# caishiqing/voice-tts

Measured on AMD Instinct MI355X. Metric: audio_seconds_per_second, higher is better.
Workload: dtype bf16

## Files before the change

### include/ixtts_hip.h

```cpp
#ifndef IXTTS_HIP_H
#define IXTTS_HIP_H

#include <stddef.h>
#include <stdint.h>

#ifdef __cplusplus
extern "C" {
#endif

#define IXTTS_OK 0
#define IXTTS_ERR_ARG (-1)
#define IXTTS_ERR_HIP (-2)
#define IXTTS_ERR_STATE (-3)
#define IXTTS_ERR_NOMEM (-4)
#define IXTTS_ERR_NAME (-5)

const char* ixtts_version(void);
const char* ixtts_last_error(void);

int ixtts_aa_snake_f32(const float* x_dev, float* y_dev, const float* up12_dev, const float* down12_dev,
                       const float* log_alpha_dev, const float* log_beta_dev, int B, int C, int T, void* stream);

size_t ixtts_attn_full_workspace_bytes(int B, int H, int T);
int ixtts_attn_full_f32(const float* q_dev, const float* k_dev, const float* v_dev, float* out_dev, int B, int H, int T,
                        int head_dim, long stride_b, long stride_t, long stride_h, long ostride_b, long ostride_t,
                        long ostride_h, float scale, void* workspace_dev, size_t workspace_bytes, void* stream);

size_t ixtts_attn_full_varlen_workspace_bytes(int nseq, int H, int total_tiles);
int ixtts_attn_full_varlen_f32(const float* q_dev, const float* k_dev, const float* v_dev, float* out_dev, const int* table_dev, int nseq,
                               int total_tiles, int n_work, int H, int head_dim, long stride_t, long stride_h, long ostride_t, long ostride_h,
                               float scale, void* workspace_dev, size_t workspace_bytes, void* stream);

int ixtts_adaln_rmsnorm_f32(const float* x_dev, const float* wb_dev, const float* g_dev, float* out_dev, int B, int T, int H, float eps,
                            void* stream);
int ixtts_ln_modulate_f32(const float* x_dev, const float* shift_scale_dev, float* out_dev, int B, int T, int H, float eps, void* stream);
int ixtts_rope_qk_f32(float* qkv_dev, const float* cos_sin_dev, int B, int T, int H, int head_dim, void* stream);
int ixtts_swiglu_f32(const float* u_dev, float* out_dev, long rows, int F, void* stream);
int ixtts_wn_gate_f32(const float* a_dev, const float* g_dev, float* out_dev, int B, int C, int T, long g_stride, int g_offset, void* stream);
int ixtts_wn_gate_rows_f32(const float* a_dev, const float* g_dev, float* out_dev, long rows, int C, long rows_per_batch, int B, long g_stride,
                           int g_offset, void* stream);
int ixtts_reflect_halo_rows_f32(float* p_dev, int B, int T, int C, int left, int right, void* stream);

int ixtts_adaln_rmsnorm_varlen_f32(const float* x_dev, const float* wb_dev, const float* g_dev, float* out_dev, const int* seq_off_dev, int nseq,
                                   long rows, int H, float eps, void* stream);
int ixtts_ln_modulate_varlen_f32(const float* x_dev, const float* shift_scale_dev, float* out_dev, const int* seq_off_dev, int nseq, long rows, int H,
                                 float eps, void* stream);
int ixtts_rope_qk_varlen_f32(float* qkv_dev, const float* cos_sin_dev, const int* seq_off_dev, int nseq, long rows, int H, int head_dim, void* stream);
int ixtts_wn_gate_rows_varlen_f32(const float* a_dev, const float* g_dev, float* out_dev, long rows, int C, const int* seq_off_dev, int nseq,
                                  long g_stride, int g_offset, void* stream);
int ixtts_reflect_halo_rows_varlen_f32(float* p_dev, const int* seq_off_dev, int nseq, int C, int left, int right, void* stream);

size_t ixtts_gemm_x6_packed_bytes(int N, int K);
int ixtts_gemm_x6_pack(const float* w_dev, void* packed_dev, int N, int K, void* stream);
long ixtts_gemm_x6_rows_padded(long rows);
int ixtts_gemm_x6_split(const float* a_dev, long lda, void* planes_dev, long rows, int K, void* stream);
int ixtts_gemm_x6_f32(const void* a_planes_dev, long rows_total, long row0, const void* packed_dev, const float* bias_dev, float* c_dev, long ldc,
                      int M, int N, int K, int accumulate, int tile, void* stream);
int ixtts_gemm_x6_pair_f32(const void* a_planes_dev, long rows_total, long row0, int taps, const void* packed_dev, const float* bias_dev,
                           const float* gate_dev, long gate_ld, long rows_per_batch, int nbatch, float* c_dev, long ldc, int M, int N, int K,
                           int epilogue, int tile, void* stream);
int ixtts_gemm_x6_pair_gate_varlen_f32(const void* a_planes_dev, long rows_total, long row0, int taps, const void* packed_dev, const float* bias_dev,
                                       const float* gate_dev, long gate_ld, const int* seq_off_dev, int nseq, float* c_dev, long ldc, int M, int N,
                                       int K, int tile, void* stream);

#define IXTTS_BIGVGAN_MAX_STAGES 8
#define IXTTS_BIGVGAN_MAX_RESK 4

typedef struct ixtts_bigvgan_cfg {
  int num_mels;
  int upsample_initial_channel;
  int n_stages;
  int upsample_rates[IXTTS_BIGVGAN_MAX_STAGES];
  int upsample_kernel_sizes[IXTTS_BIGVGAN_MAX_STAGES];
  int n_resblock_kernels;
  int resblock_kernel_sizes[IXTTS_BIGVGAN_MAX_RESK];
  int resblock_dilations[IXTTS_BIGVGAN_MAX_RESK][3];
  int max_frames;
  int fast_sin;
} ixtts_bigvgan_cfg;

typedef struct ixtts_bigvgan ixtts_bigvgan;

int ixtts_bigvgan_create(ixtts_bigvgan** out, const ixtts_bigvgan_cfg* cfg);
int ixtts_bigvgan_set_tensor(ixtts_bigvgan* h, const char* name, const float* data_host, const int64_t* shape, int ndim);
int ixtts_bigvgan_finalize(ixtts_bigvgan* h);
int ixtts_bigvgan_arena(ixtts_bigvgan* h, void** ptr_dev, size_t* bytes);
int ixtts_bigvgan_adopt_arena(ixtts_bigvgan* h);
int ixtts_bigvgan_forward(ixtts_bigvgan* h, const float* mel_dev, int B, int F, float* wav_dev, void* stream);
double ixtts_bigvgan_flops(const ixtts_bigvgan* h, int B, int F);
int ixtts_bigvgan_destroy(ixtts_bigvgan* h);

#define IXTTS_DTYPE_F32 0
#define IXTTS_DTYPE_BF16 1

typedef struct ixtts_gpt_cfg {
  int model_dim;
  int layers;
  int heads;
  int n_mel_codes;
  int n_mel_pos;
  int n_text_tokens;
  int n_text_pos;
  int start_mel_token;
  int stop_mel_token;
  int max_seq;
  int max_batch;
  int weight_dtype;
} ixtts_gpt_cfg;

typedef struct ixtts_sampler_cfg {
  float repetition_penalty;
  float temperature;
  int top_k;
  float top_p;
  int do_sample;
  int suppress_stop;
  uint64_t seed;
  float typical_mass;
  float length_penalty;
} ixtts_sampler_cfg;

typedef struct ixtts_gpt ixtts_gpt;

int ixtts_gpt_create(ixtts_gpt** out, const ixtts_gpt_cfg* cfg);
int ixtts_gpt_set_tensor(ixtts_gpt* h, const char* name, const float* data_host, const int64_t* shape, int ndim);
int ixtts_gpt_finalize(ixtts_gpt* h);
int ixtts_gpt_arena(ixtts_gpt* h, void** ptr_dev, size_t* bytes);
int ixtts_gpt_adopt_arena(ixtts_gpt* h);
int ixtts_gpt_share_arena(ixtts_gpt* h, ixtts_gpt* owner);

int ixtts_gpt_prefill(ixtts_gpt* h, int b, const float* embeds_dev, int n_rows, int n_left_pad, void* stream);
int ixtts_gpt_decode(ixtts_gpt* h, int n_active, int n_steps, const ixtts_sampler_cfg* sc, void* stream);
int ixtts_gpt_read(ixtts_gpt* h, int b, int32_t* ids_host, int cap, int* n_ids, int* finished, void* stream);
int ixtts_gpt_read_logits(ixtts_gpt* h, int b, float* logits_host, void* stream);
int ixtts_gpt_read_probs(ixtts_gpt* h, int b, float* probs_host, void* stream);
int ixtts_gpt_force_next(ixtts_gpt* h, int b, int32_t token, void* stream);

int ixtts_gpt_beam_begin(ixtts_gpt* h, int num_beams, void* stream);
int ixtts_gpt_beam_decode(ixtts_gpt* h, int n_steps, const ixtts_sampler_cfg* sc, void* stream);
int ixtts_gpt_beam_read(ixtts_gpt* h, int max_new, int32_t* ids_host, int cap, int* n_ids, int* done, float* score,
                        float* beam_scores_host, int32_t* last_tokens_host, int32_t* beam_idx_host, void* stream);
int ixtts_gpt_beam_force(ixtts_gpt* h, const int32_t* picks_host, int n, void* stream);

int ixtts_gpt_beam_begin_group(ixtts_gpt* h, int group, int num_beams, uint64_t rng_stream, void* stream);
int ixtts_gpt_beam_park_group(ixtts_gpt* h, int group, void* stream);
int ixtts_gpt_beam_decode_groups(ixtts_gpt* h, int n_groups, int n_steps, const ixtts_sampler_cfg* sc, void* stream);
int ixtts_gpt_beam_read_group(ixtts_gpt* h, int group, int max_new, int32_t* ids_host, int cap, int* n_ids, int* done, float* score,
                              float* beam_scores_host, int32_t* last_tokens_host, int32_t* beam_idx_host, void* stream);
int ixtts_gpt_beam_force_group(ixtts_gpt* h, int group, const int32_t* picks_host, int n, void* stream);

int ixtts_gpt_latent(ixtts_gpt* h, const float* prefix_dev, int n_prefix, const int32_t* codes_dev, int n,
                     float* latent_dev, void* stream);

int ixtts_gpt_bench_gemv(ixtts_gpt* h, int which, int layer, int batch, void* stream);
double ixtts_gpt_step_bytes(const ixtts_gpt* h, int B, int S);

int ixtts_gpt_max_batch(void);

int ixtts_gpt_destroy(ixtts_gpt* h);

#define IXTTS_DTYPE_F16 2
#define IXTTS_QWEN_TOPK_MAX 64
#define IXTTS_QWEN_MAX_EOS 8

typedef struct ixtts_qwen_cfg {
  int hidden_size;
  int layers;
  int heads;
  int kv_heads;
  int head_dim;
  int intermediate_size;
  int vocab_size;
  float rms_norm_eps;
  float rope_theta;
  int tie_word_embeddings;
  int max_seq;
  int weight_dtype;
  int n_eos;
  int eos_ids[IXTTS_QWEN_MAX_EOS];
} ixtts_qwen_cfg;

typedef struct ixtts_qwen_sampling {
  int do_sample;
  float temperature;
  int top_k;
  float top_p;
  uint64_t seed;
} ixtts_qwen_sampling;

typedef struct ixtts_qwen ixtts_qwen;

int ixtts_qwen_create(ixtts_qwen** out, const ixtts_qwen_cfg* cfg);
int ixtts_qwen_set_tensor(ixtts_qwen* h, const char* name, const float* data_host, const int64_t* shape, int ndim);
int ixtts_qwen_finalize(ixtts_qwen* h);
int ixtts_qwen_prefill(ixtts_qwen* h, const int32_t* ids_host, int n, void* stream);
int ixtts_qwen_step(ixtts_qwen* h, int n_steps, const ixtts_qwen_sampling* sc, void* stream);
int ixtts_qwen_read(ixtts_qwen* h, int32_t* ids_host, int cap, int* n_ids, int* finished, void* stream);
int ixtts_qwen_generate(ixtts_qwen* h, int max_new, const ixtts_qwen_sampling* sc, int32_t* ids_host, int cap, int* n_ids,
                        int* finished, void* stream);
int ixtts_qwen_read_logits(ixtts_qwen* h, float* logits_host, void* stream);
int ixtts_qwen_read_kept(ixtts_qwen* h, int32_t* ids_host, float* probs_host, int cap, int* n_kept, void* stream);
int ixtts_qwen_draw(ixtts_qwen* h, uint64_t seed, int n, int32_t* ids_host, void* stream);
double ixtts_qwen_step_bytes(const ixtts_qwen* h, int S);
int ixtts_qwen_destroy(ixtts_qwen* h);

#ifdef __cplusplus
}
#endif
#endif
```

### voice-tts_amd/_lib.py

```python
import ctypes as C
import os

HERE = os.path.dirname(os.path.abspath(__file__))
LIB_PATH = os.environ.get("IXTTS_LIB") or os.path.join(HERE, "libixtts_hip.so")

MAX_STAGES = 8
MAX_RESK = 4


class BigVGANCfg(C.Structure):
    _fields_ = [
        ("num_mels", C.c_int), ("upsample_initial_channel", C.c_int), ("n_stages", C.c_int),
        ("upsample_rates", C.c_int * MAX_STAGES), ("upsample_kernel_sizes", C.c_int * MAX_STAGES),
        ("n_resblock_kernels", C.c_int), ("resblock_kernel_sizes", C.c_int * MAX_RESK),
        ("resblock_dilations", (C.c_int * 3) * MAX_RESK), ("max_frames", C.c_int), ("fast_sin", C.c_int),
    ]


class GptCfg(C.Structure):
    _fields_ = [
        ("model_dim", C.c_int), ("layers", C.c_int), ("heads", C.c_int), ("n_mel_codes", C.c_int),
        ("n_mel_pos", C.c_int), ("n_text_tokens", C.c_int), ("n_text_pos", C.c_int),
        ("start_mel_token", C.c_int), ("stop_mel_token", C.c_int), ("max_seq", C.c_int),
        ("max_batch", C.c_int), ("weight_dtype", C.c_int),
    ]


class SamplerCfg(C.Structure):
    _fields_ = [
        ("repetition_penalty", C.c_float), ("temperature", C.c_float), ("top_k", C.c_int),
        ("top_p", C.c_float), ("do_sample", C.c_int), ("suppress_stop", C.c_int), ("seed", C.c_uint64),
        ("typical_mass", C.c_float), ("length_penalty", C.c_float),
    ]


QWEN_TOPK_MAX = 64
QWEN_MAX_EOS = 8


class QwenCfg(C.Structure):
    _fields_ = [
        ("hidden_size", C.c_int), ("layers", C.c_int), ("heads", C.c_int), ("kv_heads", C.c_int), ("head_dim", C.c_int),
        ("intermediate_size", C.c_int), ("vocab_size", C.c_int), ("rms_norm_eps", C.c_float), ("rope_theta", C.c_float),
        ("tie_word_embeddings", C.c_int), ("max_seq", C.c_int), ("weight_dtype", C.c_int), ("n_eos", C.c_int),
        ("eos_ids", C.c_int * QWEN_MAX_EOS),
    ]


class QwenSampling(C.Structure):
    _fields_ = [("do_sample", C.c_int), ("temperature", C.c_float), ("top_k", C.c_int), ("top_p", C.c_float), ("seed", C.c_uint64)]


_P = C.c_void_p
SYMBOLS = {
    "ixtts_version": (C.c_char_p, []),
    "ixtts_last_error": (C.c_char_p, []),
    "ixtts_aa_snake_f32": (C.c_int, [_P, _P, _P, _P, _P, _P, C.c_int, C.c_int, C.c_int, _P]),
    "ixtts_attn_full_workspace_bytes": (C.c_size_t, [C.c_int, C.c_int, C.c_int]),
    "ixtts_attn_full_f32": (C.c_int, [_P, _P, _P, _P, C.c_int, C.c_int, C.c_int, C.c_int, C.c_long, C.c_long, C.c_long, C.c_long, C.c_long,
                                      C.c_long, C.c_float, _P, C.c_size_t, _P]),
    "ixtts_attn_full_varlen_workspace_bytes": (C.c_size_t, [C.c_int, C.c_int, C.c_int]),
    "ixtts_attn_full_varlen_f32": (C.c_int, [_P, _P, _P, _P, _P, C.c_int, C.c_int, C.c_int, C.c_int, C.c_int, C.c_long, C.c_long, C.c_long, C.c_long,
                                             C.c_float, _P, C.c_size_t, _P]),
    "ixtts_adaln_rmsnorm_f32": (C.c_int, [_P, _P, _P, _P, C.c_int, C.c_int, C.c_int, C.c_float, _P]),
    "ixtts_ln_modulate_f32": (C.c_int, [_P, _P, _P, C.c_int, C.c_int, C.c_int, C.c_float, _P]),
    "ixtts_rope_qk_f32": (C.c_int, [_P, _P, C.c_int, C.c_int, C.c_int, C.c_int, _P]),
    "ixtts_swiglu_f32": (C.c_int, [_P, _P, C.c_long, C.c_int, _P]),
    "ixtts_wn_gate_f32": (C.c_int, [_P, _P, _P, C.c_int, C.c_int, C.c_int, C.c_long, C.c_int, _P]),
    "ixtts_wn_gate_rows_f32": (C.c_int, [_P, _P, _P, C.c_long, C.c_int, C.c_long, C.c_int, C.c_long, C.c_int, _P]),
    "ixtts_reflect_halo_rows_f32": (C.c_int, [_P, C.c_int, C.c_int, C.c_int, C.c_int, C.c_int, _P]),
    "ixtts_adaln_rmsnorm_varlen_f32": (C.c_int, [_P, _P, _P, _P, _P, C.c_int, C.c_long, C.c_int, C.c_float, _P]),
    "ixtts_ln_modulate_varlen_f32": (C.c_int, [_P, _P, _P, _P, C.c_int, C.c_long, C.c_int, C.c_float, _P]),
    "ixtts_rope_qk_varlen_f32": (C.c_int, [_P, _P, _P, C.c_int, C.c_long, C.c_int, C.c_int, _P]),
    "ixtts_wn_gate_rows_varlen_f32": (C.c_int, [_P, _P, _P, C.c_long, C.c_int, _P, C.c_int, C.c_long, C.c_int, _P]),
    "ixtts_reflect_halo_rows_varlen_f32": (C.c_int, [_P, _P, C.c_int, C.c_int, C.c_int, C.c_int, _P]),
    "ixtts_gemm_x6_packed_bytes": (C.c_size_t, [C.c_int, C.c_int]),
    "ixtts_gemm_x6_pack": (C.c_int, [_P, _P, C.c_int, C.c_int, _P]),
    "ixtts_gemm_x6_rows_padded": (C.c_long, [C.c_long]),
    "ixtts_gemm_x6_split": (C.c_int, [_P, C.c_long, _P, C.c_long, C.c_int, _P]),
    "ixtts_gemm_x6_f32": (C.c_int, [_P, C.c_long, C.c_long, _P, _P, _P, C.c_long, C.c_int, C.c_int, C.c_int, C.c_int, C.c_int, _P]),
    "ixtts_gemm_x6_pair_f32": (C.c_int, [_P, C.c_long, C.c_long, C.c_int, _P, _P, _P, C.c_long, C.c_long, C.c_int, _P, C.c_long, C.c_int, C.c_int,
                                         C.c_int, C.c_int, C.c_int, _P]),
    "ixtts_gemm_x6_pair_gate_varlen_f32": (C.c_int, [_P, C.c_long, C.c_long, C.c_int, _P, _P, _P, C.c_long, _P, C.c_int, _P, C.c_long, C.c_int, C.c_int,
                                                     C.c_int, C.c_int, _P]),
    "ixtts_bigvgan_create": (C.c_int, [C.POINTER(_P), C.POINTER(BigVGANCfg)]),
    "ixtts_bigvgan_set_tensor": (C.c_int, [_P, C.c_char_p, _P, C.POINTER(C.c_int64), C.c_int]),
    "ixtts_bigvgan_finalize": (C.c_int, [_P]),
    "ixtts_bigvgan_arena": (C.c_int, [_P, C.POINTER(_P), C.POINTER(C.c_size_t)]),
    "ixtts_bigvgan_adopt_arena": (C.c_int, [_P]),
    "ixtts_bigvgan_forward": (C.c_int, [_P, _P, C.c_int, C.c_int, _P, _P]),
    "ixtts_bigvgan_flops": (C.c_double, [_P, C.c_int, C.c_int]),
    "ixtts_bigvgan_destroy": (C.c_int, [_P]),
    "ixtts_gpt_create": (C.c_int, [C.POINTER(_P), C.POINTER(GptCfg)]),
    "ixtts_gpt_set_tensor": (C.c_int, [_P, C.c_char_p, _P, C.POINTER(C.c_int64), C.c_int]),
    "ixtts_gpt_finalize": (C.c_int, [_P]),
    "ixtts_gpt_arena": (C.c_int, [_P, C.POINTER(_P), C.POINTER(C.c_size_t)]),
    "ixtts_gpt_adopt_arena": (C.c_int, [_P]),
    "ixtts_gpt_share_arena": (C.c_int, [_P, _P]),
    "ixtts_gpt_prefill": (C.c_int, [_P, C.c_int, _P, C.c_int, C.c_int, _P]),
    "ixtts_gpt_decode": (C.c_int, [_P, C.c_int, C.c_int, C.POINTER(SamplerCfg), _P]),
    "ixtts_gpt_read": (C.c_int, [_P, C.c_int, _P, C.c_int, C.POINTER(C.c_int), C.POINTER(C.c_int), _P]),
    "ixtts_gpt_read_logits": (C.c_int, [_P, C.c_int, _P, _P]),
    "ixtts_gpt_beam_begin": (C.c_int, [_P, C.c_int, _P]),
    "ixtts_gpt_beam_decode": (C.c_int, [_P, C.c_int, C.POINTER(SamplerCfg), _P]),
    "ixtts_gpt_beam_read": (C.c_int, [_P, C.c_int, _P, C.c_int, C.POINTER(C.c_int), C.POINTER(C.c_int), C.POINTER(C.c_float), _P, _P, _P, _P]),
    "ixtts_gpt_beam_force": (C.c_int, [_P, _P, C.c_int, _P]),
    "ixtts_gpt_beam_begin_group": (C.c_int, [_P, C.c_int, C.c_int, C.c_uint64, _P]),
    "ixtts_gpt_beam_park_group": (C.c_int, [_P, C.c_int, _P]),
    "ixtts_gpt_beam_decode_groups": (C.c_int, [_P, C.c_int, C.c_int, C.POINTER(SamplerCfg), _P]),
    "ixtts_gpt_beam_read_group": (C.c_int, [_P, C.c_int, C.c_int, _P, C.c_int, C.POINTER(C.c_int), C.POINTER(C.c_int), C.POINTER(C.c_float), _P, _P, _P, _P]),
    "ixtts_gpt_beam_force_group": (C.c_int, [_P, C.c_int, _P, C.c_int, _P]),
    "ixtts_gpt_read_probs": (C.c_int, [_P, C.c_int, _P, _P]),
    "ixtts_gpt_force_next": (C.c_int, [_P, C.c_int, C.c_int32, _P]),
    "ixtts_gpt_latent": (C.c_int, [_P, _P, C.c_int, _P, C.c_int, _P, _P]),
    "ixtts_gpt_bench_gemv": (C.c_int, [_P, C.c_int, C.c_int, C.c_int, _P]),
    "ixtts_gpt_step_bytes": (C.c_double, [_P, C.c_int, C.c_int]),
    "ixtts_gpt_max_batch": (C.c_int, []),
    "ixtts_gpt_destroy": (C.c_int, [_P]),
    "ixtts_qwen_create": (C.c_int, [C.POINTER(_P), C.POINTER(QwenCfg)]),
    "ixtts_qwen_set_tensor": (C.c_int, [_P, C.c_char_p, _P, C.POINTER(C.c_int64), C.c_int]),
    "ixtts_qwen_finalize": (C.c_int, [_P]),
    "ixtts_qwen_prefill": (C.c_int, [_P, _P, C.c_int, _P]),
    "ixtts_qwen_step": (C.c_int, [_P, C.c_int, C.POINTER(QwenSampling), _P]),
    "ixtts_qwen_read": (C.c_int, [_P, _P, C.c_int, C.POINTER(C.c_int), C.POINTER(C.c_int), _P]),
    "ixtts_qwen_generate": (C.c_int, [_P, C.c_int, C.POINTER(QwenSampling), _P, C.c_int, C.POINTER(C.c_int), C.POINTER(C.c_int), _P]),
    "ixtts_qwen_read_logits": (C.c_int, [_P, _P, _P]),
    "ixtts_qwen_read_kept": (C.c_int, [_P, _P, _P, C.c_int, C.POINTER(C.c_int), _P]),
    "ixtts_qwen_draw": (C.c_int, [_P, C.c_uint64, C.c_int, _P, _P]),
    "ixtts_qwen_step_bytes": (C.c_double, [_P, C.c_int]),
    "ixtts_qwen_destroy": (C.c_int, [_P]),
}

_lib = None


class IxttsError(RuntimeError):
    pass


def lib():
    global _lib
    if _lib is not None:
        return _lib
    import torch

    if not os.path.exists(LIB_PATH):
        raise IxttsError(
            f"{LIB_PATH} not found: build it with `python -m voice_tts_amd.build` "
            "(there is no CPU fallback for the HIP path)")
    L = C.CDLL(LIB_PATH)
    for name, (res, args) in SYMBOLS.items():
        fn = getattr(L, name)
        fn.restype = res
        fn.argtypes = args
    _lib = L
    return L


def check(rc, what=""):
    if rc != 0:
        msg = lib().ixtts_last_error().decode(errors="replace")
        raise IxttsError(f"{what} failed with code {rc}: {msg}")


def max_batch():
    return int(lib().ixtts_gpt_max_batch())


def current_stream_ptr():
    import torch

    return C.c_void_p(torch.cuda.current_stream().cuda_stream)
```

### voice-tts_amd/csrc/attn_full.h

```cpp
#pragma once
#include "common.h"

namespace ixtts {

constexpr int AF_D = 64;
constexpr int AF_KT = 64;
constexpr int AF_QW = 32;
constexpr int AF_WAVES = 4;
constexpr int AF_KSPLIT = 4;
constexpr int AX_KSPLIT = 5;

struct AttnFullArgs {
  const float* q;
  const float* k;
  const float* v;
  float* o;
  long sb, st, sh;
  long osb, ost, osh;
  int B, H, T;
  float scale;
  float* ws_o;
  float* ws_ml;
  const int* vl_tab;
  int vl_n, vl_tiles;
};

size_t attn_full_x3_plane_bytes(int B, int H, int T);
int launch_attn_full_x3(const AttnFullArgs& a, void* planes, bool split, hipStream_t st);
int launch_attn_full_x3_varlen(const AttnFullArgs& a, void* planes, int n_work, hipStream_t st);

}
```

### voice-tts_amd/csrc/attn_full.hip

```cpp
#include "attn_full.h"

namespace ixtts {

typedef float f32x16 __attribute__((ext_vector_type(16)));

constexpr int AF_KP = AF_D + 4;

template <int KSPLIT>
__global__ __launch_bounds__(AF_WAVES * 64) void attn_full_f32_kernel(AttnFullArgs a) {
  __shared__ __attribute__((aligned(16))) float Ks[AF_KT * AF_KP];
  __shared__ __attribute__((aligned(16))) float Vs[AF_KT * AF_D];
  const int bh = blockIdx.y, b = bh / a.H, h = bh % a.H;
  const int lane = threadIdx.x & 63, wave = threadIdx.x >> 6;
  const int l31 = lane & 31, lh = lane >> 5;
  const int q0 = blockIdx.x * (AF_WAVES * AF_QW) + wave * AF_QW;
  const float* qb = a.q + b * a.sb + h * a.sh;
  const float* kb = a.k + b * a.sb + h * a.sh;
  const float* vb = a.v + b * a.sb + h * a.sh;

  float qr[AF_D / 2];
  {
    const int qi = min(q0 + l31, a.T - 1);
    const float* qp = qb + (long)qi * a.st + 4 * lh;
    const float qs = a.scale * 1.4426950408889634f;
#pragma unroll
    for (int m = 0; m < AF_D / 8; ++m) {
      const float4 t = *reinterpret_cast<const float4*>(qp + 8 * m);
      qr[4 * m] = t.x * qs; qr[4 * m + 1] = t.y * qs; qr[4 * m + 2] = t.z * qs; qr[4 * m + 3] = t.w * qs;
    }
  }
  f32x16 ot[2];
#pragma unroll
  for (int j = 0; j < 2; ++j)
#pragma unroll
    for (int r = 0; r < 16; ++r) ot[j][r] = 0.f;
  float m_run = -INFINITY, l_run = 0.f;

  const int n_tiles = (a.T + AF_KT - 1) / AF_KT;
  const int tiles_per = (n_tiles + KSPLIT - 1) / KSPLIT;
  const int t_lo = (KSPLIT > 1 ? blockIdx.z * tiles_per : 0) * AF_KT;
  const int t_hi = KSPLIT > 1 ? min(a.T, t_lo + tiles_per * AF_KT) : a.T;
  for (int t0 = t_lo; t0 < t_hi; t0 += AF_KT) {
    __syncthreads();
#pragma unroll
    for (int i = 0; i < (AF_KT * AF_D / 4) / (AF_WAVES * 64); ++i) {
      const int idx = threadIdx.x + i * (AF_WAVES * 64);
      const int key = idx >> 4, c4 = idx & 15;
      const int t = min(t0 + key, a.T - 1);
      const float4 kv = *reinterpret_cast<const float4*>(kb + (long)t * a.st + c4 * 4);
      const float4 vv = *reinterpret_cast<const float4*>(vb + (long)t * a.st + c4 * 4);
      *reinterpret_cast<float4*>(Ks + key * AF_KP + c4 * 4) = kv;
      *reinterpret_cast<float4*>(Vs + key * AF_D + c4 * 4) = vv;
    }
    __syncthreads();

    f32x16 st[2];
#pragma unroll
    for (int j = 0; j < 2; ++j)
#pragma unroll
      for (int r = 0; r < 16; ++r) st[j][r] = 0.f;
    const float* kp0 = Ks + l31 * AF_KP + 4 * lh;
    const float* kp1 = kp0 + 32 * AF_KP;
    float4 ka[2][2];
    ka[0][0] = *reinterpret_cast<const float4*>(kp0);
    ka[0][1] = *reinterpret_cast<const float4*>(kp1);
#pragma unroll
    for (int m = 0; m < AF_D / 8; ++m) {
      if (m + 1 < AF_D / 8) {
        ka[(m + 1) & 1][0] = *reinterpret_cast<const float4*>(kp0 + 8 * (m + 1));
        ka[(m + 1) & 1][1] = *reinterpret_cast<const float4*>(kp1 + 8 * (m + 1));
      }
#pragma unroll
      for (int j = 0; j < 2; ++j) {
        const float4 kk4 = ka[m & 1][j];
        st[j] = __builtin_amdgcn_mfma_f32_32x32x2f32(kk4.x, qr[4 * m], st[j], 0, 0, 0);
        st[j] = __builtin_amdgcn_mfma_f32_32x32x2f32(kk4.y, qr[4 * m + 1], st[j], 0, 0, 0);
        st[j] = __builtin_amdgcn_mfma_f32_32x32x2f32(kk4.z, qr[4 * m + 2], st[j], 0, 0, 0);
        st[j] = __builtin_amdgcn_mfma_f32_32x32x2f32(kk4.w, qr[4 * m + 3], st[j], 0, 0, 0);
      }
    }
    if (t0 + AF_KT > a.T) {
#pragma unroll
      for (int j = 0; j < 2; ++j)
#pragma unroll
        for (int r = 0; r < 16; ++r) {
          const int key = t0 + j * 32 + (r & 3) + 8 * (r >> 2) + 4 * lh;
          if (key >= a.T) st[j][r] = -INFINITY;
        }
    }
    float tmax = -INFINITY;
#pragma unroll
    for (int j = 0; j < 2; ++j)
#pragma unroll
      for (int r = 0; r < 16; ++r) tmax = fmaxf(tmax, st[j][r]);
    tmax = fmaxf(tmax, __shfl_xor(tmax, 32, 64));
    const float mn = fmaxf(m_run, tmax);
    const float alpha = __builtin_amdgcn_exp2f(m_run - mn);
    m_run = mn;
    if (alpha != 1.0f) {
#pragma unroll
      for (int j = 0; j < 2; ++j)
#pragma unroll
        for (int r = 0; r < 16; ++r) ot[j][r] *= alpha;
    }
    float psum = 0.f;
    const float* vp = Vs + (4 * lh) * AF_D + l31;
    float va[2][2];
    va[0][0] = vp[0];
    va[0][1] = vp[32];
#pragma unroll
    for (int s = 0; s < 32; ++s) {
      const int j = s >> 4, r = s & 15;
      if (s + 1 < 32) {
        const int j1 = (s + 1) >> 4, r1 = (s + 1) & 15;
        const float* vrow = vp + (j1 * 32 + (r1 & 3) + 8 * (r1 >> 2)) * AF_D;
        va[(s + 1) & 1][0] = vrow[0];
        va[(s + 1) & 1][1] = vrow[32];
      }
      const float pv = __builtin_amdgcn_exp2f(st[j][r] - mn);
      psum += pv;
      ot[0] = __builtin_amdgcn_mfma_f32_32x32x2f32(va[s & 1][0], pv, ot[0], 0, 0, 0);
      ot[1] = __builtin_amdgcn_mfma_f32_32x32x2f32(va[s & 1][1], pv, ot[1], 0, 0, 0);
    }
    psum += __shfl_xor(psum, 32, 64);
    l_run = l_run * alpha + psum;
  }
  const int qi = q0 + l31;
  if (qi < a.T) {
    if constexpr (KSPLIT == 1) {
      const float inv = 1.0f / l_run;
      float* op = a.o + b * a.osb + (long)qi * a.ost + h * a.osh;
#pragma unroll
      for (int j = 0; j < 2; ++j)
#pragma unroll
        for (int r = 0; r < 16; ++r) op[j * 32 + (r & 3) + 8 * (r >> 2) + 4 * lh] = ot[j][r] * inv;
    } else {
      const long row = ((long)blockIdx.z * a.B * a.H + bh) * a.T + qi;
      float* op = a.ws_o + row * AF_D;
#pragma unroll
      for (int j = 0; j < 2; ++j)
#pragma unroll
        for (int r = 0; r < 16; ++r) op[j * 32 + (r & 3) + 8 * (r >> 2) + 4 * lh] = ot[j][r];
      if (lh == 0) *reinterpret_cast<float2*>(a.ws_ml + row * 2) = make_float2(m_run, l_run);
    }
  }
}

template <int KSPLIT>
__global__ __launch_bounds__(256) void attn_full_merge_kernel(AttnFullArgs a) {
  const long row = (long)blockIdx.x * 4 + (threadIdx.x >> 6);
  const long rows = (long)a.B * a.H * a.T;
  if (row >= rows) return;
  const int d = threadIdx.x & 63;
  const int t = (int)(row % a.T);
  const int bh = (int)(row / a.T), b = bh / a.H, h = bh % a.H;
  float2 ml[KSPLIT];
  float o[KSPLIT];
  float M = -INFINITY;
#pragma unroll
  for (int sp = 0; sp < KSPLIT; ++sp) {
    ml[sp] = *reinterpret_cast<const float2*>(a.ws_ml + ((long)sp * rows + row) * 2);
    o[sp] = a.ws_o[((long)sp * rows + row) * AF_D + d];
    M = fmaxf(M, ml[sp].x);
  }
  float L = 0.f, O = 0.f;
#pragma unroll
  for (int sp = 0; sp < KSPLIT; ++sp) {
    const float w = (ml[sp].x > -INFINITY) ? __builtin_amdgcn_exp2f(ml[sp].x - M) : 0.f;
    L = fmaf(ml[sp].y, w, L);
    O = fmaf(o[sp], w, O);
  }
  a.o[b * a.osb + (long)t * a.ost + h * a.osh + d] = O / L;
}

}

static size_t attn_partials_bytes(int B, int H, int T) {
  return (size_t)(ixtts::AF_KSPLIT > ixtts::AX_KSPLIT ? ixtts::AF_KSPLIT : ixtts::AX_KSPLIT) * B * H * T * (ixtts::AF_D + 2) * sizeof(float);
}

extern "C" size_t ixtts_attn_full_workspace_bytes(int B, int H, int T) {
  if (B <= 0 || H <= 0 || T <= 0) return 0;
  return attn_partials_bytes(B, H, T) + ixtts::attn_full_x3_plane_bytes(B, H, T);
}

extern "C" int ixtts_attn_full_f32(const float* q_dev, const float* k_dev, const float* v_dev, float* out_dev, int B, int H, int T,
                                   int head_dim, long stride_b, long stride_t, long stride_h, long ostride_b, long ostride_t,
                                   long ostride_h, float scale, void* workspace_dev, size_t workspace_bytes, void* stream) {
  using namespace ixtts;
  IX_ARG(q_dev && k_dev && v_dev && out_dev, "attn_full: null pointer");
  IX_ARG(head_dim == AF_D, "attn_full: head_dim %d (only 64 is built)", head_dim);
  IX_ARG(B > 0 && H > 0 && T > 0 && (long)B * H <= 65535, "attn_full: bad shape B=%d H=%d T=%d", B, H, T);
  IX_ARG(stride_t % 4 == 0 && stride_h % 4 == 0 && stride_b % 4 == 0, "attn_full: strides must keep 16-byte row alignment");
  AttnFullArgs a;
  a.q = q_dev; a.k = k_dev; a.v = v_dev; a.o = out_dev;
  a.sb = stride_b; a.st = stride_t; a.sh = stride_h;
  a.osb = ostride_b; a.ost = ostride_t; a.osh = ostride_h;
  a.B = B; a.H = H; a.T = T; a.scale = scale;
  a.ws_o = a.ws_ml = nullptr;
  a.vl_tab = nullptr; a.vl_n = a.vl_tiles = 0;
  hipStream_t st = (hipStream_t)stream;
  const int qblocks = ceil_div(T, AF_WAVES * AF_QW);
  const bool have_ws = workspace_dev && workspace_bytes >= ixtts_attn_full_workspace_bytes(B, H, T);
  const bool split = have_ws && T > 4 * AF_KT && (long)qblocks * B * H * AF_WAVES < 2 * 1024;
  const char* mode = getenv("IXTTS_ATTN_FULL");
  const bool x3 = !(mode && strcmp(mode, "f32") == 0);
  const bool use_x3 = x3 && have_ws;
  if (split) {
    a.ws_o = reinterpret_cast<float*>(workspace_dev);
    a.ws_ml = a.ws_o + (size_t)(use_x3 ? AX_KSPLIT : AF_KSPLIT) * B * H * T * AF_D;
  }
  if (use_x3) {
    IX_TRY(launch_attn_full_x3(a, reinterpret_cast<char*>(workspace_dev) + attn_partials_bytes(B, H, T), split, st));
    if (split) {
      const long rows = (long)B * H * T;
      hipLaunchKernelGGL(attn_full_merge_kernel<AX_KSPLIT>, dim3((unsigned)((rows + 3) / 4)), dim3(256), 0, st, a);
    }
    IX_HIP(hipGetLastError());
    return IXTTS_OK;
  }
  if (split) {
    hipLaunchKernelGGL(attn_full_f32_kernel<AF_KSPLIT>, dim3(qblocks, B * H, AF_KSPLIT), dim3(AF_WAVES * 64), 0, st, a);
    const long rows = (long)B * H * T;
    hipLaunchKernelGGL(attn_full_merge_kernel<AF_KSPLIT>, dim3((unsigned)((rows + 3) / 4)), dim3(256), 0, st, a);
  } else {
    hipLaunchKernelGGL(attn_full_f32_kernel<1>, dim3(qblocks, B * H), dim3(AF_WAVES * 64), 0, st, a);
  }
  IX_HIP(hipGetLastError());
  return IXTTS_OK;
}

extern "C" size_t ixtts_attn_full_varlen_workspace_bytes(int nseq, int H, int total_tiles) {
  if (nseq <= 0 || H <= 0 || total_tiles <= 0) return 0;
  return (size_t)H * total_tiles * 2 * 3 * 8 * 64 * 16;
}

extern "C" int ixtts_attn_full_varlen_f32(const float* q_dev, const float* k_dev, const float* v_dev, float* out_dev, const int* table_dev, int nseq,
                                          int total_tiles, int n_work, int H, int head_dim, long stride_t, long stride_h, long ostride_t, long ostride_h,
                                          float scale, void* workspace_dev, size_t workspace_bytes, void* stream) {
  using namespace ixtts;
  IX_ARG(q_dev && k_dev && v_dev && out_dev && table_dev, "attn_full_varlen: null pointer");
  IX_ARG(head_dim == AF_D, "attn_full_varlen: head_dim %d (only 64 is built)", head_dim);
  IX_ARG(nseq > 0 && total_tiles >= nseq && n_work >= nseq && H > 0 && H <= 65535, "attn_full_varlen: bad shape nseq=%d tiles=%d work=%d H=%d", nseq, total_tiles,
         n_work, H);
  IX_ARG(stride_t % 4 == 0 && stride_h % 4 == 0, "attn_full_varlen: strides must keep 16-byte row alignment");
  IX_ARG(workspace_dev && workspace_bytes >= ixtts_attn_full_varlen_workspace_bytes(nseq, H, total_tiles), "attn_full_varlen: workspace of %zu bytes, %zu needed",
         workspace_bytes, ixtts_attn_full_varlen_workspace_bytes(nseq, H, total_tiles));
  AttnFullArgs a;
  a.q = q_dev; a.k = k_dev; a.v = v_dev; a.o = out_dev;
  a.sb = 0; a.st = stride_t; a.sh = stride_h;
  a.osb = 0; a.ost = ostride_t; a.osh = ostride_h;
  a.B = 1; a.H = H; a.T = 0; a.scale = scale;
  a.ws_o = a.ws_ml = nullptr;
  a.vl_tab = table_dev; a.vl_n = nseq; a.vl_tiles = total_tiles;
  return launch_attn_full_x3_varlen(a, workspace_dev, n_work, (hipStream_t)stream);
}
```

### voice-tts_amd/csrc/attn_full_x3.hip

```cpp
#include "attn_full.h"

namespace ixtts {

typedef float ax_f32x16 __attribute__((ext_vector_type(16)));
typedef __bf16 ax_bf16x8 __attribute__((ext_vector_type(8)));

constexpr int AX_TILE_UNITS = 3 * 8 * 64;
constexpr int AX_WAVES = 4;

size_t attn_full_x3_plane_bytes(int B, int H, int T) {
  const size_t tiles = (size_t)(T + AF_KT - 1) / AF_KT;
  return (size_t)B * H * tiles * 2 * AX_TILE_UNITS * 16;
}


template <bool VL>
__global__ __launch_bounds__(256) void attn_kv_planes_kernel(AttnFullArgs a, uint4* __restrict__ planes) {
  int tile = blockIdx.x, T = a.T;
  const float *kb, *vb;
  uint4* kdst;
  if constexpr (VL) {
    const int h = blockIdx.y, s = seq_of_row(a.vl_tab + a.vl_n + 1, a.vl_n, tile);
    const int r0 = a.vl_tab[s];
    T = a.vl_tab[s + 1] - r0;
    kdst = planes + ((size_t)h * a.vl_tiles + tile) * 2 * AX_TILE_UNITS;
    tile -= a.vl_tab[a.vl_n + 1 + s];
    kb = a.k + (long)r0 * a.st + h * a.sh;
    vb = a.v + (long)r0 * a.st + h * a.sh;
  } else {
    const int bh = blockIdx.y, b = bh / a.H, h = bh % a.H;
    const int n_tiles = (a.T + AF_KT - 1) / AF_KT;
    kb = a.k + b * a.sb + h * a.sh;
    vb = a.v + b * a.sb + h * a.sh;
    kdst = planes + ((size_t)bh * n_tiles + tile) * 2 * AX_TILE_UNITS;
  }
  uint4* vdst = kdst + AX_TILE_UNITS;
  const int t0 = tile * AF_KT;
#pragma unroll
  for (int i = 0; i < 2; ++i) {
    const int uid = threadIdx.x + 256 * i;
    const int key = uid >> 3, oct = uid & 7;
    const int t = t0 + key;
    float v[8];
    const float4* src = reinterpret_cast<const float4*>(kb + (long)min(t, T - 1) * a.st + 8 * oct);
    const float4 x0 = src[0], x1 = src[1];
    const bool live = t < T;
    v[0] = live ? x0.x : 0.f; v[1] = live ? x0.y : 0.f; v[2] = live ? x0.z : 0.f; v[3] = live ? x0.w : 0.f;
    v[4] = live ? x1.x : 0.f; v[5] = live ? x1.y : 0.f; v[6] = live ? x1.z : 0.f; v[7] = live ? x1.w : 0.f;
    uint4 ph, pm, pl;
    split8_bf16x3(v, ph, pm, pl);
    kdst[(0 * 8 + oct) * 64 + key] = ph;
    kdst[(1 * 8 + oct) * 64 + key] = pm;
    kdst[(2 * 8 + oct) * 64 + key] = pl;
  }
#pragma unroll
  for (int i = 0; i < 2; ++i) {
    const int d = threadIdx.x & 63, un = (threadIdx.x >> 6) + 4 * i;
    const int j = un >> 2, u = (un >> 1) & 1, kh = un & 1;
    float v[8];
#pragma unroll
    for (int e = 0; e < 8; ++e) {
      const int t = t0 + 32 * j + 16 * u + 8 * (e >> 2) + 4 * kh + (e & 3);
      const float x = vb[(long)min(t, T - 1) * a.st + d];
      v[e] = t < T ? x : 0.f;
    }
    uint4 ph, pm, pl;
    split8_bf16x3(v, ph, pm, pl);
    vdst[(0 * 8 + un) * 64 + d] = ph;
    vdst[(1 * 8 + un) * 64 + d] = pm;
    vdst[(2 * 8 + un) * 64 + d] = pl;
  }
}

template <int KSPLIT, bool VL = false>
__global__ __launch_bounds__(AX_WAVES * 64, 3) void attn_full_x3_kernel(AttnFullArgs a, const uint4* __restrict__ planes) {
  __shared__ uint4 Ks[AX_TILE_UNITS];
  __shared__ uint4 Vs[AX_TILE_UNITS];
  static_assert(!VL || KSPLIT == 1, "packed sequences: no key-range split");
  const int lane = threadIdx.x & 63, wave = threadIdx.x >> 6;
  const int l31 = lane & 31, lh = lane >> 5;
  int T, q0;
  const float* qb;
  const uint4* pb;
  float* ob;
  if constexpr (VL) {
    const int h = blockIdx.y;
    const int* w = a.vl_tab + 2 * (a.vl_n + 1) + 2 * blockIdx.x;
    const int s = w[0], r0 = a.vl_tab[s];
    T = a.vl_tab[s + 1] - r0;
    q0 = w[1] * (AX_WAVES * AF_QW) + wave * AF_QW;
    qb = a.q + (long)r0 * a.st + h * a.sh;
    pb = planes + ((size_t)h * a.vl_tiles + a.vl_tab[a.vl_n + 1 + s]) * 2 * AX_TILE_UNITS;
    ob = a.o + (long)r0 * a.ost + h * a.osh;
  } else {
    const int bh = blockIdx.y, b = bh / a.H, h = bh % a.H;
    T = a.T;
    q0 = blockIdx.x * (AX_WAVES * AF_QW) + wave * AF_QW;
    qb = a.q + b * a.sb + h * a.sh;
    pb = planes + (size_t)bh * ((T + AF_KT - 1) / AF_KT) * 2 * AX_TILE_UNITS;
    ob = a.o + b * a.osb + h * a.osh;
  }

  uint4 qp[4][3];
  {
    const int qi = min(q0 + l31, T - 1);
    const float* qrow = qb + (long)qi * a.st + 8 * lh;
    const float qs = a.scale * 1.4426950408889634f;
#pragma unroll
    for (int s = 0; s < 4; ++s) {
      const float4 x0 = *reinterpret_cast<const float4*>(qrow + 16 * s), x1 = *reinterpret_cast<const float4*>(qrow + 16 * s + 4);
      const float v[8] = {x0.x * qs, x0.y * qs, x0.z * qs, x0.w * qs, x1.x * qs, x1.y * qs, x1.z * qs, x1.w * qs};
      split8_bf16x3(v, qp[s][0], qp[s][1], qp[s][2]);
    }
  }
  ax_f32x16 ot[2];
#pragma unroll
  for (int j = 0; j < 2; ++j)
#pragma unroll
    for (int r = 0; r < 16; ++r) ot[j][r] = 0.f;
  float m_run = -INFINITY, l_run = 0.f;

  const int n_tiles = (T + AF_KT - 1) / AF_KT;
  const int tiles_per = (n_tiles + KSPLIT - 1) / KSPLIT;
  const int tile_lo = KSPLIT > 1 ? blockIdx.z * tiles_per : 0;
  const int tile_hi = KSPLIT > 1 ? min(n_tiles, tile_lo + tiles_per) : n_tiles;
  auto issue_tile = [&](const uint4* __restrict__ src, uint4* __restrict__ dst) {
#pragma unroll
    for (int i = 0; i < AX_TILE_UNITS / (AX_WAVES * 64); ++i)
      __builtin_amdgcn_global_load_lds((const __attribute__((address_space(1))) void*)(src + i * (AX_WAVES * 64) + threadIdx.x),
                                       (__attribute__((address_space(3))) void*)(dst + i * (AX_WAVES * 64) + wave * 64), 16, 0, 0);
  };
  auto mfma6x2 = [](ax_f32x16& c0, ax_f32x16& c1, const uint4 (&A0)[3], const uint4 (&A1)[3], const uint4 (&Bq)[3]) {
    const ax_bf16x8 a0h = __builtin_bit_cast(ax_bf16x8, A0[0]), a0m = __builtin_bit_cast(ax_bf16x8, A0[1]), a0l = __builtin_bit_cast(ax_bf16x8, A0[2]);
    const ax_bf16x8 a1h = __builtin_bit_cast(ax_bf16x8, A1[0]), a1m = __builtin_bit_cast(ax_bf16x8, A1[1]), a1l = __builtin_bit_cast(ax_bf16x8, A1[2]);
    const ax_bf16x8 bh_ = __builtin_bit_cast(ax_bf16x8, Bq[0]), bm = __builtin_bit_cast(ax_bf16x8, Bq[1]), bl = __builtin_bit_cast(ax_bf16x8, Bq[2]);
    c0 = __builtin_amdgcn_mfma_f32_32x32x16_bf16(a0l, bh_, c0, 0, 0, 0);
    c1 = __builtin_amdgcn_mfma_f32_32x32x16_bf16(a1l, bh_, c1, 0, 0, 0);
    c0 = __builtin_amdgcn_mfma_f32_32x32x16_bf16(a0h, bl, c0, 0, 0, 0);
    c1 = __builtin_amdgcn_mfma_f32_32x32x16_bf16(a1h, bl, c1, 0, 0, 0);
    c0 = __builtin_amdgcn_mfma_f32_32x32x16_bf16(a0m, bm, c0, 0, 0, 0);
    c1 = __builtin_amdgcn_mfma_f32_32x32x16_bf16(a1m, bm, c1, 0, 0, 0);
    c0 = __builtin_amdgcn_mfma_f32_32x32x16_bf16(a0m, bh_, c0, 0, 0, 0);
    c1 = __builtin_amdgcn_mfma_f32_32x32x16_bf16(a1m, bh_, c1, 0, 0, 0);
    c0 = __builtin_amdgcn_mfma_f32_32x32x16_bf16(a0h, bm, c0, 0, 0, 0);
    c1 = __builtin_amdgcn_mfma_f32_32x32x16_bf16(a1h, bm, c1, 0, 0, 0);
    c0 = __builtin_amdgcn_mfma_f32_32x32x16_bf16(a0h, bh_, c0, 0, 0, 0);
    c1 = __builtin_amdgcn_mfma_f32_32x32x16_bf16(a1h, bh_, c1, 0, 0, 0);
  };
  if (tile_lo < tile_hi) issue_tile(pb + (size_t)tile_lo * 2 * AX_TILE_UNITS, Ks);
  for (int tile = tile_lo; tile < tile_hi; ++tile) {
    const int t0 = tile * AF_KT;
    asm volatile("s_waitcnt vmcnt(0)" ::: "memory");
    __builtin_amdgcn_s_barrier();
    issue_tile(pb + ((size_t)tile * 2 + 1) * AX_TILE_UNITS, Vs);
    ax_f32x16 st[2];
#pragma unroll
    for (int j = 0; j < 2; ++j)
#pragma unroll
      for (int r = 0; r < 16; ++r) st[j][r] = 0.f;
    const uint4* kp = Ks + lh * 64 + l31;
#pragma unroll
    for (int s = 0; s < 4; ++s) {
      uint4 ka[2][3];
#pragma unroll
      for (int j = 0; j < 2; ++j)
#pragma unroll
        for (int pl = 0; pl < 3; ++pl) ka[j][pl] = kp[(pl * 8 + 2 * s) * 64 + 32 * j];
      mfma6x2(st[0], st[1], ka[0], ka[1], qp[s]);
    }
    if (t0 + AF_KT > T) {
#pragma unroll
      for (int j = 0; j < 2; ++j)
#pragma unroll
        for (int r = 0; r < 16; ++r) {
          const int key = t0 + j * 32 + (r & 3) + 8 * (r >> 2) + 4 * lh;
          if (key >= T) st[j][r] = -INFINITY;
        }
    }
    float tmax = -INFINITY;
#pragma unroll
    for (int j = 0; j < 2; ++j)
#pragma unroll
      for (int r = 0; r < 16; ++r) tmax = fmaxf(tmax, st[j][r]);
    tmax = fmaxf(tmax, __shfl_xor(tmax, 32, 64));
    const float mn = fmaxf(m_run, tmax);
    const float alpha = __builtin_amdgcn_exp2f(m_run - mn);
    m_run = mn;
    if (alpha != 1.0f) {
#pragma unroll
      for (int j = 0; j < 2; ++j)
#pragma unroll
        for (int r = 0; r < 16; ++r) ot[j][r] *= alpha;
    }
    float psum = 0.f;
#pragma unroll
    for (int j = 0; j < 2; ++j)
#pragma unroll
      for (int r = 0; r < 16; ++r) {
        st[j][r] = __builtin_amdgcn_exp2f(st[j][r] - mn);
        psum += st[j][r];
      }
    psum += __shfl_xor(psum, 32, 64);
    l_run = l_run * alpha + psum;
    asm volatile("s_waitcnt vmcnt(0)" ::: "memory");
    __builtin_amdgcn_s_barrier();
    if (tile + 1 < tile_hi) issue_tile(pb + (size_t)(tile + 1) * 2 * AX_TILE_UNITS, Ks);
    const uint4* vp = Vs + lh * 64 + l31;
#pragma unroll
    for (int s = 0; s < 4; ++s) {
      const int j = s >> 1, u = s & 1;
      uint4 va[2][3];
#pragma unroll
      for (int dh = 0; dh < 2; ++dh)
#pragma unroll
        for (int pl = 0; pl < 3; ++pl) va[dh][pl] = vp[(pl * 8 + 2 * s) * 64 + 32 * dh];
      uint4 pp[3];
      {
        float pv[8];
#pragma unroll
        for (int e = 0; e < 8; ++e) pv[e] = st[j][8 * u + e];
        split8_bf16x3(pv, pp[0], pp[1], pp[2]);
      }
      mfma6x2(ot[0], ot[1], va[0], va[1], pp);
    }
  }
  asm volatile("s_waitcnt vmcnt(0)" ::: "memory");
  const int qi = q0 + l31;
  if (qi < T) {
    if constexpr (KSPLIT == 1) {
      const float inv = 1.0f / l_run;
      float* op = ob + (long)qi * a.ost;
#pragma unroll
      for (int j = 0; j < 2; ++j)
#pragma unroll
        for (int r = 0; r < 16; ++r) op[j * 32 + (r & 3) + 8 * (r >> 2) + 4 * lh] = ot[j][r] * inv;
    } else {
      const long row = ((long)blockIdx.z * a.B * a.H + blockIdx.y) * T + qi;
      float* op = a.ws_o + row * AF_D;
#pragma unroll
      for (int j = 0; j < 2; ++j)
#pragma unroll
        for (int r = 0; r < 16; ++r) op[j * 32 + (r & 3) + 8 * (r >> 2) + 4 * lh] = ot[j][r];
      if (lh == 0) *reinterpret_cast<float2*>(a.ws_ml + row * 2) = make_float2(m_run, l_run);
    }
  }
}

int launch_attn_full_x3(const AttnFullArgs& a, void* planes, bool split, hipStream_t st) {
  const int n_tiles = ceil_div(a.T, AF_KT);
  const int qblocks = ceil_div(a.T, AX_WAVES * AF_QW);
  uint4* pl = reinterpret_cast<uint4*>(planes);
  hipLaunchKernelGGL(attn_kv_planes_kernel<false>, dim3(n_tiles, a.B * a.H), dim3(256), 0, st, a, pl);
  if (split) hipLaunchKernelGGL(attn_full_x3_kernel<AX_KSPLIT>, dim3(qblocks, a.B * a.H, AX_KSPLIT), dim3(AX_WAVES * 64), 0, st, a, (const uint4*)pl);
  else hipLaunchKernelGGL(attn_full_x3_kernel<1>, dim3(qblocks, a.B * a.H), dim3(AX_WAVES * 64), 0, st, a, (const uint4*)pl);
  IX_HIP(hipGetLastError());
  return IXTTS_OK;
}

int launch_attn_full_x3_varlen(const AttnFullArgs& a, void* planes, int n_work, hipStream_t st) {
  uint4* pl = reinterpret_cast<uint4*>(planes);
  hipLaunchKernelGGL(attn_kv_planes_kernel<true>, dim3(a.vl_tiles, a.H), dim3(256), 0, st, a, pl);
  hipLaunchKernelGGL((attn_full_x3_kernel<1, true>), dim3(n_work, a.H), dim3(AX_WAVES * 64), 0, st, a, (const uint4*)pl);
  IX_HIP(hipGetLastError());
  return IXTTS_OK;
}

}
```

### voice-tts_amd/csrc/common.h

```cpp
#pragma once
#include <type_traits>
#include <hip/hip_runtime.h>
#include <hip/hip_bf16.h>
#include <stdint.h>
#include <stdio.h>
#include <string.h>
#include <string>

#include "../../include/ixtts_hip.h"

namespace ixtts {

void set_error(const char* fmt, ...);

#define IX_HIP(expr)                                                                   \
  do {                                                                                 \
    hipError_t _e = (expr);                                                            \
    if (_e != hipSuccess) {                                                            \
      ::ixtts::set_error("%s:%d: %s -> %s", __FILE__, __LINE__, #expr, hipGetErrorString(_e)); \
      return IXTTS_ERR_HIP;                                                            \
    }                                                                                  \
  } while (0)

#define IX_ARG(cond, ...)                  \
  do {                                     \
    if (!(cond)) {                         \
      ::ixtts::set_error(__VA_ARGS__);     \
      return IXTTS_ERR_ARG;                \
    }                                      \
  } while (0)

#define IX_TRY(expr)            \
  do {                          \
    int _r = (expr);            \
    if (_r != IXTTS_OK) return _r; \
  } while (0)

static inline int ceil_div(int a, int b) { return (a + b - 1) / b; }
static inline size_t align_up(size_t x, size_t a) { return (x + a - 1) / a * a; }

typedef __hip_bfloat16 bf16;

__device__ __forceinline__ float bf16_bits_to_f32(unsigned short b) {
  return __uint_as_float(((unsigned int)b) << 16);
}
__device__ __forceinline__ int seq_of_row(const int* __restrict__ off, int n, long row) {
  int lo = 0, hi = n - 1;
  while (lo < hi) {
    const int mid = (lo + hi + 1) >> 1;
    if ((long)off[mid] <= row) lo = mid;
    else hi = mid - 1;
  }
  return lo;
}

__device__ __forceinline__ float lo_bf16(unsigned int w) { return __uint_as_float(w << 16); }
__device__ __forceinline__ float hi_bf16(unsigned int w) { return __uint_as_float(w & 0xffff0000u); }

template <int CTRL, int ROW_MASK, int BANK_MASK>
__device__ __forceinline__ float dpp_take(float v) {
  return __builtin_bit_cast(float, __builtin_amdgcn_update_dpp(0, __builtin_bit_cast(int, v), CTRL, ROW_MASK, BANK_MASK, true));
}
__device__ __forceinline__ float wave_sum63(float v) {
  float s = v + dpp_take<0x111, 0xf, 0xf>(v);
  s += dpp_take<0x112, 0xf, 0xf>(v);
  s += dpp_take<0x113, 0xf, 0xf>(v);
  s += dpp_take<0x114, 0xf, 0xe>(s);
  s += dpp_take<0x118, 0xf, 0xc>(s);
  s += dpp_take<0x142, 0xa, 0xf>(s);
  s += dpp_take<0x143, 0xc, 0xf>(s);
  return s;
}
__device__ __forceinline__ float wave_sum(float v) {
  return __builtin_bit_cast(float, __builtin_amdgcn_readlane(__builtin_bit_cast(int, wave_sum63(v)), 63));
}
__device__ __forceinline__ float wave_max(float v) {
#pragma unroll
  for (int o = 32; o >= 1; o >>= 1) v = fmaxf(v, __shfl_xor(v, o, 64));
  return v;
}
template <int CTRL, int ROW_MASK, int BANK_MASK>
__device__ __forceinline__ float dpp_take_or_self(float v) {
  return __builtin_bit_cast(float, __builtin_amdgcn_update_dpp(__builtin_bit_cast(int, v), __builtin_bit_cast(int, v), CTRL, ROW_MASK, BANK_MASK, false));
}
__device__ __forceinline__ float wave_max_dpp(float v) {
  float s = fmaxf(v, dpp_take_or_self<0x111, 0xf, 0xf>(v));
  s = fmaxf(s, dpp_take_or_self<0x112, 0xf, 0xf>(v));
  s = fmaxf(s, dpp_take_or_self<0x113, 0xf, 0xf>(v));
  s = fmaxf(s, dpp_take_or_self<0x114, 0xf, 0xe>(s));
  s = fmaxf(s, dpp_take_or_self<0x118, 0xf, 0xc>(s));
  s = fmaxf(s, dpp_take_or_self<0x142, 0xa, 0xf>(s));
  s = fmaxf(s, dpp_take_or_self<0x143, 0xc, 0xf>(s));
  return __builtin_bit_cast(float, __builtin_amdgcn_readlane(__builtin_bit_cast(int, s), 63));
}
__device__ __forceinline__ unsigned int wave_scan_u32(unsigned int v) {
  auto take = [](unsigned int x, auto ctrl, auto rm, auto bm) {
    return (unsigned int)__builtin_amdgcn_update_dpp(0, (int)x, decltype(ctrl)::value, decltype(rm)::value, decltype(bm)::value, true);
  };
  using std::integral_constant;
  unsigned int s = v + take(v, integral_constant<int, 0x111>{}, integral_constant<int, 0xf>{}, integral_constant<int, 0xf>{});
  s += take(v, integral_constant<int, 0x112>{}, integral_constant<int, 0xf>{}, integral_constant<int, 0xf>{});
  s += take(v, integral_constant<int, 0x113>{}, integral_constant<int, 0xf>{}, integral_constant<int, 0xf>{});
  s += take(s, integral_constant<int, 0x114>{}, integral_constant<int, 0xf>{}, integral_constant<int, 0xe>{});
  s += take(s, integral_constant<int, 0x118>{}, integral_constant<int, 0xf>{}, integral_constant<int, 0xc>{});
  s += take(s, integral_constant<int, 0x142>{}, integral_constant<int, 0xa>{}, integral_constant<int, 0xf>{});
  s += take(s, integral_constant<int, 0x143>{}, integral_constant<int, 0xc>{}, integral_constant<int, 0xf>{});
  return s;
}

__device__ __forceinline__ int wave_min_i32_dpp(int v) {
  auto take = [](int x, auto ctrl, auto rm, auto bm) {
    return __builtin_amdgcn_update_dpp(x, x, decltype(ctrl)::value, decltype(rm)::value, decltype(bm)::value, false);
  };
  using std::integral_constant;
  int s = min(v, take(v, integral_constant<int, 0x111>{}, integral_constant<int, 0xf>{}, integral_constant<int, 0xf>{}));
  s = min(s, take(v, integral_constant<int, 0x112>{}, integral_constant<int, 0xf>{}, integral_constant<int, 0xf>{}));
  s = min(s, take(v, integral_constant<int, 0x113>{}, integral_constant<int, 0xf>{}, integral_constant<int, 0xf>{}));
  s = min(s, take(s, integral_constant<int, 0x114>{}, integral_constant<int, 0xf>{}, integral_constant<int, 0xe>{}));
  s = min(s, take(s, integral_constant<int, 0x118>{}, integral_constant<int, 0xf>{}, integral_constant<int, 0xc>{}));
  s = min(s, take(s, integral_constant<int, 0x142>{}, integral_constant<int, 0xa>{}, integral_constant<int, 0xf>{}));
  s = min(s, take(s, integral_constant<int, 0x143>{}, integral_constant<int, 0xc>{}, integral_constant<int, 0xf>{}));
  return __builtin_amdgcn_readlane(s, 63);
}

__device__ __forceinline__ void split8_bf16x3(const float (&v)[8], uint4& ph, uint4& pm, uint4& pl) {
  unsigned int h[8], m[8], l[8];
#pragma unroll
  for (int e = 0; e < 8; ++e) {
    h[e] = __float_as_uint(v[e]) + 0x8000u;
    const float r = v[e] - __uint_as_float(h[e] & 0xffff0000u);
    m[e] = __float_as_uint(r) + 0x8000u;
    l[e] = __float_as_uint(r - __uint_as_float(m[e] & 0xffff0000u));
  }
  auto pk = [](unsigned int hi, unsigned int lo) { return __builtin_amdgcn_perm(hi, lo, 0x07060302u); };
  ph = make_uint4(pk(h[1], h[0]), pk(h[3], h[2]), pk(h[5], h[4]), pk(h[7], h[6]));
  pm = make_uint4(pk(m[1], m[0]), pk(m[3], m[2]), pk(m[5], m[4]), pk(m[7], m[6]));
  pl = make_uint4(pk(l[1], l[0]), pk(l[3], l[2]), pk(l[5], l[4]), pk(l[7], l[6]));
}

}
```

### voice-tts_amd/csrc/dit_ops.hip

```cpp
#include "common.h"

namespace ixtts {

constexpr int ROW_NV = 8;

template <bool CENTER>
__global__ __launch_bounds__(256) void row_norm_mod_kernel(const float* __restrict__ x, const float* __restrict__ mw, const float* __restrict__ mb,
                                                           const float* __restrict__ g, float* __restrict__ out, long rows, int T, int H, long mstride,
                                                           float eps, float wadd, const int* __restrict__ seq_off = nullptr, int nseq = 0) {
  const long row = (long)blockIdx.x * 4 + (threadIdx.x >> 6);
  if (row >= rows) return;
  const int lane = threadIdx.x & 63;
  const int H4 = H >> 2;
  const float4* xr = reinterpret_cast<const float4*>(x + row * H);
  float4 v[ROW_NV];
#pragma unroll
  for (int i = 0; i < ROW_NV; ++i) {
    const int c = lane + 64 * i;
    v[i] = (c < H4) ? xr[c] : make_float4(0.f, 0.f, 0.f, 0.f);
  }
  float mean = 0.f;
  if constexpr (CENTER) {
    float s = 0.f;
#pragma unroll
    for (int i = 0; i < ROW_NV; ++i) s += (v[i].x + v[i].y) + (v[i].z + v[i].w);
    mean = wave_sum(s) / (float)H;
  }
  float q = 0.f;
#pragma unroll
  for (int i = 0; i < ROW_NV; ++i) {
    const int c = lane + 64 * i;
    if (c < H4) {
      const float a = v[i].x - mean, b = v[i].y - mean, cc = v[i].z - mean, d = v[i].w - mean;
      q += (a * a + b * b) + (cc * cc + d * d);
    }
  }
  const float rstd = 1.0f / sqrtf(wave_sum(q) / (float)H + eps);
  const long bidx = seq_off ? seq_of_row(seq_off, nseq, row) : row / T;
  const float4* w4 = reinterpret_cast<const float4*>(mw + bidx * mstride);
  const float4* b4 = reinterpret_cast<const float4*>(mb + bidx * mstride);
  const float4* g4 = reinterpret_cast<const float4*>(g);
  float4* o4 = reinterpret_cast<float4*>(out + row * H);
#pragma unroll
  for (int i = 0; i < ROW_NV; ++i) {
    const int c = lane + 64 * i;
    if (c < H4) {
      const float4 w = w4[c], b = b4[c];
      float4 n = make_float4((v[i].x - mean) * rstd, (v[i].y - mean) * rstd, (v[i].z - mean) * rstd, (v[i].w - mean) * rstd);
      if (g) {
        const float4 gg = g4[c];
        n.x *= gg.x; n.y *= gg.y; n.z *= gg.z; n.w *= gg.w;
      }
      o4[c] = make_float4(fmaf(w.x + wadd, n.x, b.x), fmaf(w.y + wadd, n.y, b.y), fmaf(w.z + wadd, n.z, b.z), fmaf(w.w + wadd, n.w, b.w));
    }
  }
}

__global__ __launch_bounds__(256) void rope_qk_kernel(float* __restrict__ qkv, const float2* __restrict__ tab, long rows, int T, int H, int hd,
                                                      const int* __restrict__ seq_off = nullptr, int nseq = 0) {
  const int per_row = (2 * H) >> 2;
  const long idx = (long)blockIdx.x * 256 + threadIdx.x;
  if (idx >= rows * per_row) return;
  const long row = idx / per_row;
  const int c4 = (int)(idx % per_row);
  const int col = c4 * 4;
  const int t = seq_off ? (int)(row - seq_off[seq_of_row(seq_off, nseq, row)]) : (int)(row % T);
  const int p = (col % hd) >> 1;
  float4* ptr = reinterpret_cast<float4*>(qkv + row * 3 * H + col);
  const float4 v = *ptr;
  const float2 f0 = tab[(long)t * (hd >> 1) + p], f1 = tab[(long)t * (hd >> 1) + p + 1];
  *ptr = make_float4(v.x * f0.x - v.y * f0.y, v.y * f0.x + v.x * f0.y, v.z * f1.x - v.w * f1.y, v.w * f1.x + v.z * f1.y);
}

__global__ __launch_bounds__(256) void swiglu_kernel(const float* __restrict__ u, float* __restrict__ out, long rows, int Fd) {
  const int F4 = Fd >> 2;
  const long idx = (long)blockIdx.x * 256 + threadIdx.x;
  if (idx >= rows * F4) return;
  const long row = idx / F4;
  const int c = (int)(idx % F4);
  const float4 a = reinterpret_cast<const float4*>(u + row * 2 * Fd)[c];
  const float4 b = reinterpret_cast<const float4*>(u + row * 2 * Fd + Fd)[c];
  auto f = [](float x, float y) { return x / (1.0f + expf(-x)) * y; };
  reinterpret_cast<float4*>(out + row * Fd)[c] = make_float4(f(a.x, b.x), f(a.y, b.y), f(a.z, b.z), f(a.w, b.w));
}

__global__ __launch_bounds__(256) void wn_gate_kernel(const float* __restrict__ a, const float* __restrict__ gvec, float* __restrict__ out, int B, int C, int T,
                                                      long gstride, int goff) {
  const long idx = (long)blockIdx.x * 256 + threadIdx.x;
  const long n = (long)B * C * T;
  if (idx >= n) return;
  const int t = (int)(idx % T);
  const int c = (int)((idx / T) % C);
  const int b = (int)(idx / ((long)T * C));
  const float ga = gvec[b * gstride + goff + c], gb = gvec[b * gstride + goff + C + c];
  const float xa = a[((long)b * 2 * C + c) * T + t] + ga;
  const float xb = a[((long)b * 2 * C + C + c) * T + t] + gb;
  out[idx] = tanhf(xa) * (1.0f / (1.0f + expf(-xb)));
}

__global__ __launch_bounds__(256) void wn_gate_rows_kernel(const float* __restrict__ a, const float* __restrict__ gvec, float* __restrict__ out, long rows, int C,
                                                           long rows_per_batch, int B, long gstride, int goff, const int* __restrict__ seq_off = nullptr) {
  const long idx = (long)blockIdx.x * 256 + threadIdx.x;
  const int C4 = C >> 2;
  if (idx >= rows * C4) return;
  const long r = idx / C4;
  const int c = (int)(idx % C4) * 4;
  const int b = seq_off ? seq_of_row(seq_off, B, r) : (int)min(r / rows_per_batch, (long)B - 1);
  const float4 xa = *reinterpret_cast<const float4*>(a + r * 2 * C + c);
  const float4 xb = *reinterpret_cast<const float4*>(a + r * 2 * C + C + c);
  const float4 ga = *reinterpret_cast<const float4*>(gvec + b * gstride + goff + c);
  const float4 gb = *reinterpret_cast<const float4*>(gvec + b * gstride + goff + C + c);
  float4 o;
  o.x = tanhf(xa.x + ga.x) * (1.0f / (1.0f + expf(-(xb.x + gb.x))));
  o.y = tanhf(xa.y + ga.y) * (1.0f / (1.0f + expf(-(xb.y + gb.y))));
  o.z = tanhf(xa.z + ga.z) * (1.0f / (1.0f + expf(-(xb.z + gb.z))));
  o.w = tanhf(xa.w + ga.w) * (1.0f / (1.0f + expf(-(xb.w + gb.w))));
  *reinterpret_cast<float4*>(out + r * C + c) = o;
}

__global__ __launch_bounds__(256) void reflect_halo_rows_kernel(float* __restrict__ p, int B, int T, int C, int left, int right) {
  const int C4 = C >> 2;
  const long idx = (long)blockIdx.x * 256 + threadIdx.x;
  const long per_b = (long)(left + right) * C4;
  if (idx >= per_b * B) return;
  const int b = (int)(idx / per_b);
  const int h = (int)((idx % per_b) / C4);
  const int c = (int)(idx % C4) * 4;
  float* base = p + (long)b * (left + T + right) * C;
  const int dst = h < left ? left - 1 - h : left + T + (h - left);
  const int src = h < left ? left + h + 1 : left + T - 2 - (h - left);
  *reinterpret_cast<float4*>(base + (long)dst * C + c) = *reinterpret_cast<const float4*>(base + (long)src * C + c);
}

__global__ __launch_bounds__(256) void reflect_halo_rows_varlen_kernel(float* __restrict__ p, const int* __restrict__ off, int n, int C, int left, int right) {
  const int C4 = C >> 2;
  const long idx = (long)blockIdx.x * 256 + threadIdx.x;
  const long per_b = (long)(left + right) * C4;
  if (idx >= per_b * n) return;
  const int b = (int)(idx / per_b);
  const int h = (int)((idx % per_b) / C4);
  const int c = (int)(idx % C4) * 4;
  const int o0 = off[b], T = off[b + 1] - o0 - left - right;
  if (T <= left || T <= right) return;
  float* base = p + (long)o0 * C;
  const int dst = h < left ? left - 1 - h : left + T + (h - left);
  const int src = h < left ? left + h + 1 : left + T - 2 - (h - left);
  *reinterpret_cast<float4*>(base + (long)dst * C + c) = *reinterpret_cast<const float4*>(base + (long)src * C + c);
}

}

using namespace ixtts;

extern "C" int ixtts_adaln_rmsnorm_f32(const float* x_dev, const float* wb_dev, const float* g_dev, float* out_dev, int B, int T, int H, float eps,
                                       void* stream) {
  IX_ARG(x_dev && wb_dev && g_dev && out_dev, "adaln_rmsnorm: null pointer");
  IX_ARG(B > 0 && T > 0 && H > 0 && H % 4 == 0 && H <= 64 * ROW_NV * 4, "adaln_rmsnorm: bad shape B=%d T=%d H=%d", B, T, H);
  const long rows = (long)B * T;
  hipLaunchKernelGGL(row_norm_mod_kernel<false>, dim3((unsigned)((rows + 3) / 4)), dim3(256), 0, (hipStream_t)stream, x_dev, wb_dev, wb_dev + H, g_dev, out_dev,
                     rows, T, H, (long)2 * H, eps, 0.0f);
  IX_HIP(hipGetLastError());
  return IXTTS_OK;
}

extern "C" int ixtts_ln_modulate_f32(const float* x_dev, const float* shift_scale_dev, float* out_dev, int B, int T, int H, float eps, void* stream) {
  IX_ARG(x_dev && shift_scale_dev && out_dev, "ln_modulate: null pointer");
  IX_ARG(B > 0 && T > 0 && H > 0 && H % 4 == 0 && H <= 64 * ROW_NV * 4, "ln_modulate: bad shape B=%d T=%d H=%d", B, T, H);
  const long rows = (long)B * T;
  hipLaunchKernelGGL(row_norm_mod_kernel<true>, dim3((unsigned)((rows + 3) / 4)), dim3(256), 0, (hipStream_t)stream, x_dev, shift_scale_dev + H, shift_scale_dev,
                     (const float*)nullptr, out_dev, rows, T, H, (long)2 * H, eps, 1.0f);
  IX_HIP(hipGetLastError());
  return IXTTS_OK;
}

extern "C" int ixtts_rope_qk_f32(float* qkv_dev, const float* cos_sin_dev, int B, int T, int H, int head_dim, void* stream) {
  IX_ARG(qkv_dev && cos_sin_dev, "rope_qk: null pointer");
  IX_ARG(B > 0 && T > 0 && H > 0 && head_dim > 0 && head_dim % 4 == 0 && H % head_dim == 0, "rope_qk: bad shape B=%d T=%d H=%d hd=%d", B, T, H, head_dim);
  const long n = (long)B * T * (2 * H / 4);
  hipLaunchKernelGGL(rope_qk_kernel, dim3((unsigned)((n + 255) / 256)), dim3(256), 0, (hipStream_t)stream, qkv_dev, reinterpret_cast<const float2*>(cos_sin_dev),
                     (long)B * T, T, H, head_dim);
  IX_HIP(hipGetLastError());
  return IXTTS_OK;
}

extern "C" int ixtts_swiglu_f32(const float* u_dev, float* out_dev, long rows, int F, void* stream) {
  IX_ARG(u_dev && out_dev, "swiglu: null pointer");
  IX_ARG(rows > 0 && F > 0 && F % 4 == 0, "swiglu: bad shape rows=%ld F=%d", rows, F);
  const long n = rows * (F / 4);
  hipLaunchKernelGGL(swiglu_kernel, dim3((unsigned)((n + 255) / 256)), dim3(256), 0, (hipStream_t)stream, u_dev, out_dev, rows, F);
  IX_HIP(hipGetLastError());
  return IXTTS_OK;
}

extern "C" int ixtts_wn_gate_f32(const float* a_dev, const float* g_dev, float* out_dev, int B, int C, int T, long g_stride, int g_offset, void* stream) {
  IX_ARG(a_dev && g_dev && out_dev, "wn_gate: null pointer");
  IX_ARG(B > 0 && C > 0 && T > 0 && g_offset >= 0, "wn_gate: bad shape B=%d C=%d T=%d", B, C, T);
  const long n = (long)B * C * T;
  hipLaunchKernelGGL(wn_gate_kernel, dim3((unsigned)((n + 255) / 256)), dim3(256), 0, (hipStream_t)stream, a_dev, g_dev, out_dev, B, C, T, g_stride, g_offset);
  IX_HIP(hipGetLastError());
  return IXTTS_OK;
}

extern "C" int ixtts_wn_gate_rows_f32(const float* a_dev, const float* g_dev, float* out_dev, long rows, int C, long rows_per_batch, int B, long g_stride,
                                      int g_offset, void* stream) {
  IX_ARG(a_dev && g_dev && out_dev, "wn_gate_rows: null pointer");
  IX_ARG(rows > 0 && C > 0 && C % 4 == 0 && rows_per_batch > 0 && B > 0 && g_offset >= 0 && g_offset % 4 == 0 && g_stride % 4 == 0,
         "wn_gate_rows: bad shape rows=%ld C=%d rows_per_batch=%ld B=%d", rows, C, rows_per_batch, B);
  const long n = rows * (C / 4);
  hipLaunchKernelGGL(wn_gate_rows_kernel, dim3((unsigned)((n + 255) / 256)), dim3(256), 0, (hipStream_t)stream, a_dev, g_dev, out_dev, rows, C, rows_per_batch, B,
                     g_stride, g_offset);
  IX_HIP(hipGetLastError());
  return IXTTS_OK;
}

extern "C" int ixtts_reflect_halo_rows_f32(float* p_dev, int B, int T, int C, int left, int right, void* stream) {
  IX_ARG(p_dev, "reflect_halo_rows: null pointer");
  IX_ARG(B > 0 && C > 0 && C % 4 == 0 && left >= 0 && right >= 0 && T > left && T > right, "reflect_halo_rows: bad shape B=%d T=%d C=%d left=%d right=%d", B, T, C,
         left, right);
  const long n = (long)B * (left + right) * (C / 4);
  if (n == 0) return IXTTS_OK;
  hipLaunchKernelGGL(reflect_halo_rows_kernel, dim3((unsigned)((n + 255) / 256)), dim3(256), 0, (hipStream_t)stream, p_dev, B, T, C, left, right);
  IX_HIP(hipGetLastError());
  return IXTTS_OK;
}


extern "C" int ixtts_adaln_rmsnorm_varlen_f32(const float* x_dev, const float* wb_dev, const float* g_dev, float* out_dev, const int* seq_off_dev, int nseq,
                                              long rows, int H, float eps, void* stream) {
  IX_ARG(x_dev && wb_dev && g_dev && out_dev && seq_off_dev, "adaln_rmsnorm_varlen: null pointer");
  IX_ARG(nseq > 0 && rows > 0 && H > 0 && H % 4 == 0 && H <= 64 * ROW_NV * 4, "adaln_rmsnorm_varlen: bad shape nseq=%d rows=%ld H=%d", nseq, rows, H);
  hipLaunchKernelGGL(row_norm_mod_kernel<false>, dim3((unsigned)((rows + 3) / 4)), dim3(256), 0, (hipStream_t)stream, x_dev, wb_dev, wb_dev + H, g_dev, out_dev,
                     rows, 1, H, (long)2 * H, eps, 0.0f, seq_off_dev, nseq);
  IX_HIP(hipGetLastError());
  return IXTTS_OK;
}

extern "C" int ixtts_ln_modulate_varlen_f32(const float* x_dev, const float* shift_scale_dev, float* out_dev, const int* seq_off_dev, int nseq, long rows, int H,
                                            float eps, void* stream) {
  IX_ARG(x_dev && shift_scale_dev && out_dev && seq_off_dev, "ln_modulate_varlen: null pointer");
  IX_ARG(nseq > 0 && rows > 0 && H > 0 && H % 4 == 0 && H <= 64 * ROW_NV * 4, "ln_modulate_varlen: bad shape nseq=%d rows=%ld H=%d", nseq, rows, H);
  hipLaunchKernelGGL(row_norm_mod_kernel<true>, dim3((unsigned)((rows + 3) / 4)), dim3(256), 0, (hipStream_t)stream, x_dev, shift_scale_dev + H, shift_scale_dev,
                     (const float*)nullptr, out_dev, rows, 1, H, (long)2 * H, eps, 1.0f, seq_off_dev, nseq);
  IX_HIP(hipGetLastError());
  return IXTTS_OK;
}

extern "C" int ixtts_rope_qk_varlen_f32(float* qkv_dev, const float* cos_sin_dev, const int* seq_off_dev, int nseq, long rows, int H, int head_dim, void* stream) {
  IX_ARG(qkv_dev && cos_sin_dev && seq_off_dev, "rope_qk_varlen: null pointer");
  IX_ARG(nseq > 0 && rows > 0 && H > 0 && head_dim > 0 && head_dim % 4 == 0 && H % head_dim == 0, "rope_qk_varlen: bad shape nseq=%d rows=%ld H=%d hd=%d", nseq,
         rows, H, head_dim);
  const long n = rows * (2 * H / 4);
  hipLaunchKernelGGL(rope_qk_kernel, dim3((unsigned)((n + 255) / 256)), dim3(256), 0, (hipStream_t)stream, qkv_dev, reinterpret_cast<const float2*>(cos_sin_dev),
                     rows, 1, H, head_dim, seq_off_dev, nseq);
  IX_HIP(hipGetLastError());
  return IXTTS_OK;
}

extern "C" int ixtts_wn_gate_rows_varlen_f32(const float* a_dev, const float* g_dev, float* out_dev, long rows, int C, const int* seq_off_dev, int nseq,
                                             long g_stride, int g_offset, void* stream) {
  IX_ARG(a_dev && g_dev && out_dev && seq_off_dev, "wn_gate_rows_varlen: null pointer");
  IX_ARG(rows > 0 && C > 0 && C % 4 == 0 && nseq > 0 && g_offset >= 0 && g_offset % 4 == 0 && g_stride % 4 == 0,
         "wn_gate_rows_varlen: bad shape rows=%ld C=%d nseq=%d", rows, C, nseq);
  const long n = rows * (C / 4);
  hipLaunchKernelGGL(wn_gate_rows_kernel, dim3((unsigned)((n + 255) / 256)), dim3(256), 0, (hipStream_t)stream, a_dev, g_dev, out_dev, rows, C, (long)1, nseq,
                     g_stride, g_offset, seq_off_dev);
  IX_HIP(hipGetLastError());
  return IXTTS_OK;
}

extern "C" int ixtts_reflect_halo_rows_varlen_f32(float* p_dev, const int* seq_off_dev, int nseq, int C, int left, int right, void* stream) {
  IX_ARG(p_dev && seq_off_dev, "reflect_halo_rows_varlen: null pointer");
  IX_ARG(nseq > 0 && C > 0 && C % 4 == 0 && left >= 0 && right >= 0, "reflect_halo_rows_varlen: bad shape nseq=%d C=%d left=%d right=%d", nseq, C, left, right);
  const long n = (long)nseq * (left + right) * (C / 4);
  if (n == 0) return IXTTS_OK;
  hipLaunchKernelGGL(reflect_halo_rows_varlen_kernel, dim3((unsigned)((n + 255) / 256)), dim3(256), 0, (hipStream_t)stream, p_dev, seq_off_dev, nseq, C, left,
                     right);
  IX_HIP(hipGetLastError());
  return IXTTS_OK;
}
```

### voice-tts_amd/gemm.py

```python
import ctypes as C

import torch

from . import _lib


class PackedLinear:

    __slots__ = ("N", "K", "packed", "bias")

    def __init__(self, weight, bias=None):
        assert weight.is_cuda and weight.dim() == 2 and weight.shape[1] % 64 == 0, tuple(weight.shape)
        w = weight.detach().to(torch.float32).contiguous()
        self.N, self.K = int(w.shape[0]), int(w.shape[1])
        nbytes = _lib.lib().ixtts_gemm_x6_packed_bytes(self.N, self.K)
        self.packed = torch.empty(nbytes, dtype=torch.uint8, device=w.device)
        with torch.cuda.device(w.device):
            _lib.check(_lib.lib().ixtts_gemm_x6_pack(w.data_ptr(), self.packed.data_ptr(), self.N, self.K, _lib.current_stream_ptr()), "ixtts_gemm_x6_pack")
            torch.cuda.current_stream().synchronize()
        self.bias = None if bias is None else bias.detach().to(w.device, torch.float32).contiguous()


class Planes:

    __slots__ = ("buf", "rows", "K")

    def __init__(self, buf, rows, K):
        self.buf, self.rows, self.K = buf, rows, K


_POOL = {}


def usable(x, K):
    return x.is_cuda and x.dtype == torch.float32 and K % 64 == 0 and x.shape[-1] == K and x.stride(-1) == 1 and x.data_ptr() % 16 == 0 and \
        (x.dim() == 1 or (x.stride(-2) % 4 == 0 and x.stride(-2) >= K))


def split(x, slot=0):
    K = int(x.shape[-1])
    if x.dim() != 2:
        x = x.reshape(-1, K) if x.is_contiguous() else x.contiguous().reshape(-1, K)
    rows, lda = int(x.shape[0]), int(x.stride(0))
    L = _lib.lib()
    nbytes = (K // 16) * 6 * int(L.ixtts_gemm_x6_rows_padded(rows)) * 16
    key = (x.device, nbytes, slot)
    buf = _POOL.get(key)
    if buf is None:
        buf = _POOL[key] = torch.empty(nbytes, dtype=torch.uint8, device=x.device)
    with torch.cuda.device(x.device):
        _lib.check(L.ixtts_gemm_x6_split(x.data_ptr(), lda, buf.data_ptr(), rows, K, _lib.current_stream_ptr()), "ixtts_gemm_x6_split")
    return Planes(buf, rows, K)


def linear(x, pl, out=None, accumulate=False, bias=True, tile=0, row0=0, rows=None, lead=None):
    K, N = pl.K, pl.N
    if not isinstance(x, Planes):
        lead = tuple(x.shape[:-1]) if lead is None else lead
        x = split(x)
    assert x.K == K, (x.K, K)
    M = (x.rows - row0) if rows is None else int(rows)
    if out is None:
        assert not accumulate
        out = torch.empty(*(lead if lead is not None else (M,)), N, dtype=torch.float32, device=pl.packed.device)
    assert out.shape[-1] == N and out.stride(-1) == 1 and out.numel() >= M * N
    ldc = int(out.stride(-2)) if out.dim() >= 2 else N
    b = pl.bias if (bias and pl.bias is not None) else None
    with torch.cuda.device(pl.packed.device):
        rc = _lib.lib().ixtts_gemm_x6_f32(x.buf.data_ptr(), x.rows, int(row0), pl.packed.data_ptr(), b.data_ptr() if b is not None else None, out.data_ptr(), ldc,
                                          M, N, K, 1 if accumulate else 0, int(tile), _lib.current_stream_ptr())
    _lib.check(rc, "ixtts_gemm_x6_f32")
    return out


SWIGLU, GATE = 1, 2


def interleave_halves(a, b):
    F = a.shape[0]
    assert b.shape == a.shape and F % 32 == 0, (tuple(a.shape), tuple(b.shape))
    return torch.stack([a.reshape(F // 32, 32, *a.shape[1:]), b.reshape(F // 32, 32, *b.shape[1:])], 1).reshape(2 * F, *a.shape[1:]).contiguous()


def pair_linear(x, pl, epilogue, taps=1, out=None, gate=None, gate_off=0, rows_per_batch=1, row0=0, rows=None, tile=0, seq_off=None):
    if not isinstance(x, Planes):
        x = split(x)
    assert pl.K == taps * x.K and pl.N % 64 == 0, (pl.K, taps, x.K, pl.N)
    M = (x.rows - row0 - (taps - 1)) if rows is None else int(rows)
    if out is None:
        out = torch.empty(M, pl.N // 2, dtype=torch.float32, device=pl.packed.device)
    assert out.shape[-1] == pl.N // 2 and out.stride(-1) == 1 and out.numel() >= M * (pl.N // 2)
    ldc = int(out.stride(-2)) if out.dim() >= 2 else pl.N // 2
    gp, gld, nb = None, 0, 1
    if epilogue == GATE:
        assert gate.is_contiguous() and gate.dim() == 2 and gate_off + pl.N <= gate.shape[1]
        gp, gld, nb = gate.data_ptr() + 4 * int(gate_off), int(gate.shape[1]), int(gate.shape[0])
    b = pl.bias
    if seq_off is not None:
        assert epilogue == GATE and seq_off.tab.is_cuda and gate.shape[0] >= seq_off.n
        with torch.cuda.device(pl.packed.device):
            rc = _lib.lib().ixtts_gemm_x6_pair_gate_varlen_f32(x.buf.data_ptr(), x.rows, int(row0), int(taps), pl.packed.data_ptr(),
                                                               b.data_ptr() if b is not None else None, gp, gld, seq_off.tab.data_ptr(), int(seq_off.n),
                                                               out.data_ptr(), ldc, M, pl.N, pl.K, int(tile), _lib.current_stream_ptr())
        _lib.check(rc, "ixtts_gemm_x6_pair_gate_varlen_f32")
        return out
    with torch.cuda.device(pl.packed.device):
        rc = _lib.lib().ixtts_gemm_x6_pair_f32(x.buf.data_ptr(), x.rows, int(row0), int(taps), pl.packed.data_ptr(), b.data_ptr() if b is not None else None,
                                               gp, gld, int(rows_per_batch), nb, out.data_ptr(), ldc, M, pl.N, pl.K, int(epilogue), int(tile),
                                               _lib.current_stream_ptr())
    _lib.check(rc, "ixtts_gemm_x6_pair_f32")
    return out
```

### voice-tts_amd/s2mel.py

```python
import math
import os

import torch
import torch.nn.functional as F

from . import gemm as G
from .convs import conv1d

from .weights import fold_weight_norm

S2MEL_CFG = dict(
    hidden_dim=512, num_heads=8, depth=13, in_channels=80, content_dim=512, style_dim=192,
    wavenet_hidden=512, wavenet_layers=8, wavenet_kernel=5, wavenet_dilation_rate=1,
    lr_channels=512, lr_in_channels=1024, lr_n_blocks=4, gpt_dim=1280, codebook_dim=8, codebook_size=8192, semantic_dim=1024,
)


def tiny_s2mel_cfg(**kw):
    c = dict(S2MEL_CFG)
    c.update(hidden_dim=64, num_heads=2, depth=5, content_dim=32, style_dim=12, wavenet_hidden=64, wavenet_layers=3,
             lr_channels=32, lr_in_channels=40, lr_n_blocks=2, gpt_dim=128, codebook_size=8194, semantic_dim=40)
    c.update(kw)
    return c


def _ffn_dim(dim):
    n_hidden = int(2 * (4 * dim) / 3)
    return n_hidden if n_hidden % 256 == 0 else n_hidden + 256 - (n_hidden % 256)


def s2mel_shapes(cfg=S2MEL_CFG):
    H, Hw, C = cfg["hidden_dim"], cfg["wavenet_hidden"], cfg["in_channels"]
    assert H == Hw, "FinalLayer's adaLN takes the DiT timestep embedding: wavenet.hidden_dim must equal DiT.hidden_dim"
    out = [("gpt_layer.0.weight", (256, cfg["gpt_dim"])), ("gpt_layer.0.bias", (256,)), ("gpt_layer.1.weight", (128, 256)),
           ("gpt_layer.1.bias", (128,)), ("gpt_layer.2.weight", (cfg["semantic_dim"], 128)), ("gpt_layer.2.bias", (cfg["semantic_dim"],)),
           ("quantizer.codebook.weight", (cfg["codebook_size"], cfg["codebook_dim"])),
           ("quantizer.out_project.weight", (cfg["semantic_dim"], cfg["codebook_dim"], 1)), ("quantizer.out_project.bias", (cfg["semantic_dim"],))]
    lr = cfg["lr_channels"]
    out += [("length_regulator.content_in_proj.weight", (lr, cfg["lr_in_channels"])), ("length_regulator.content_in_proj.bias", (lr,))]
    for i in range(cfg["lr_n_blocks"]):
        out += [(f"length_regulator.model.{3 * i}.weight", (lr, lr, 3)), (f"length_regulator.model.{3 * i}.bias", (lr,)),
                (f"length_regulator.model.{3 * i + 1}.weight", (lr,)), (f"length_regulator.model.{3 * i + 1}.bias", (lr,))]
    n = 3 * cfg["lr_n_blocks"]
    out += [(f"length_regulator.model.{n}.weight", (lr, lr, 1)), (f"length_regulator.model.{n}.bias", (lr,))]
    e = "cfm.estimator."
    out += [(e + "t_embedder.mlp.0.weight", (H, 256)), (e + "t_embedder.mlp.0.bias", (H,)), (e + "t_embedder.mlp.2.weight", (H, H)), (e + "t_embedder.mlp.2.bias", (H,)),
            (e + "t_embedder2.mlp.0.weight", (Hw, 256)), (e + "t_embedder2.mlp.0.bias", (Hw,)), (e + "t_embedder2.mlp.2.weight", (Hw, Hw)), (e + "t_embedder2.mlp.2.bias", (Hw,)),
            (e + "cond_projection.weight", (H, cfg["content_dim"])), (e + "cond_projection.bias", (H,)),
            (e + "cond_x_merge_linear.weight", (H, H + 2 * C + cfg["style_dim"])), (e + "cond_x_merge_linear.bias", (H,)),
            (e + "skip_linear.weight", (H, H + C)), (e + "skip_linear.bias", (H,)),
            (e + "conv1.weight", (Hw, H)), (e + "conv1.bias", (Hw,)), (e + "conv2.weight", (C, Hw, 1)), (e + "conv2.bias", (C,)),
            (e + "res_projection.weight", (Hw, H)), (e + "res_projection.bias", (Hw,)),
            (e + "final_layer.linear.weight", (Hw, Hw)), (e + "final_layer.linear.bias", (Hw,)),
            (e + "final_layer.adaLN_modulation.1.weight", (2 * Hw, Hw)), (e + "final_layer.adaLN_modulation.1.bias", (2 * Hw,))]
    t = e + "transformer."
    inter = _ffn_dim(H)
    for i in range(cfg["depth"]):
        p = t + f"layers.{i}."
        out += [(p + "attention.wqkv.weight", (3 * H, H)), (p + "attention.wo.weight", (H, H)),
                (p + "feed_forward.w1.weight", (inter, H)), (p + "feed_forward.w3.weight", (inter, H)), (p + "feed_forward.w2.weight", (H, inter)),
                (p + "ffn_norm.project_layer.weight", (2 * H, H)), (p + "ffn_norm.project_layer.bias", (2 * H,)), (p + "ffn_norm.norm.weight", (H,)),
                (p + "attention_norm.project_layer.weight", (2 * H, H)), (p + "attention_norm.project_layer.bias", (2 * H,)), (p + "attention_norm.norm.weight", (H,)),
                (p + "skip_in_linear.weight", (H, 2 * H)), (p + "skip_in_linear.bias", (H,))]
    out += [(t + "norm.project_layer.weight", (2 * H, H)), (t + "norm.project_layer.bias", (2 * H,)), (t + "norm.norm.weight", (H,))]
    w = e + "wavenet."
    nl, k = cfg["wavenet_layers"], cfg["wavenet_kernel"]
    out += [(w + "cond_layer.conv.conv.weight", (2 * Hw * nl, Hw, 1)), (w + "cond_layer.conv.conv.bias", (2 * Hw * nl,))]
    for i in range(nl):
        rs = 2 * Hw if i < nl - 1 else Hw
        out += [(w + f"in_layers.{i}.conv.conv.weight", (2 * Hw, Hw, k)), (w + f"in_layers.{i}.conv.conv.bias", (2 * Hw,)),
                (w + f"res_skip_layers.{i}.conv.conv.weight", (rs, Hw, 1)), (w + f"res_skip_layers.{i}.conv.conv.bias", (rs,))]
    return out


def make_s2mel_weights(cfg=S2MEL_CFG, seed=1234):
    g = torch.Generator().manual_seed(seed)
    W = {}
    for name, shape in s2mel_shapes(cfg):
        if name.endswith("norm.weight") or (".model." in name and len(shape) == 1 and name.endswith(".weight")):
            W[name] = 1.0 + 0.1 * torch.randn(*shape, generator=g)
        elif name.endswith(".bias"):
            W[name] = 0.02 * torch.randn(*shape, generator=g)
        elif name == "quantizer.codebook.weight":
            W[name] = torch.randn(*shape, generator=g)
        else:
            fan = 1
            for d in shape[1:]:
                fan *= d
            W[name] = torch.randn(*shape, generator=g) / math.sqrt(fan)
    return W


def _pad_reflect(x, left, right):
    L = x.shape[-1]
    extra = 0
    if L <= max(left, right):
        extra = max(left, right) - L + 1
        x = F.pad(x, (0, extra))
    y = F.pad(x, (left, right), mode="reflect")
    return y[..., : y.shape[-1] - extra]


def attn_full(q, k, v, scale=None):
    import ctypes as C

    from . import _lib

    B, T, Hh, d = q.shape
    assert d == 64 and q.is_cuda and q.dtype == torch.float32 and k.shape == q.shape and v.shape == q.shape
    for t in (q, k, v):
        assert t.stride(3) == 1 and t.stride() == q.stride() and t.stride(1) % 4 == 0 and t.data_ptr() % 16 == 0
    out = torch.empty(B, T, Hh, d, device=q.device, dtype=torch.float32)
    sc = float(scale if scale is not None else 1.0 / math.sqrt(d))
    L = _lib.lib()
    nws = L.ixtts_attn_full_workspace_bytes(B, Hh, T)
    ws = torch.empty(nws, device=q.device, dtype=torch.uint8)
    with torch.cuda.device(q.device):
        rc = L.ixtts_attn_full_f32(q.data_ptr(), k.data_ptr(), v.data_ptr(), out.data_ptr(), B, Hh, T, d, q.stride(0), q.stride(1),
                                   q.stride(2), out.stride(0), out.stride(1), out.stride(2), C.c_float(sc), ws.data_ptr(), nws,
                                   _lib.current_stream_ptr())
    _lib.check(rc, "ixtts_attn_full_f32")
    return out


def _lin(x, W, name):
    return F.linear(x, W[name + ".weight"], W.get(name + ".bias"))


def _hip_call(name, *args):
    from . import _lib

    _lib.check(getattr(_lib.lib(), name)(*args, _lib.current_stream_ptr()), name)


def adaln_rmsnorm(x, wb, g, eps=1e-5):
    B, T, H = x.shape
    if x.is_cuda:
        import ctypes as C

        x, wb = x.contiguous(), wb.contiguous()
        out = torch.empty_like(x)
        with torch.cuda.device(x.device):
            _hip_call("ixtts_adaln_rmsnorm_f32", x.data_ptr(), wb.data_ptr(), g.data_ptr(), out.data_ptr(), B, T, H, C.c_float(eps))
        return out
    w, b = wb[:, None, :H], wb[:, None, H:]
    return torch.addcmul(b, w, F.rms_norm(x, (H,), g, eps))


def ln_modulate(x, ss, eps=1e-6):
    B, T, H = x.shape
    if x.is_cuda:
        import ctypes as C

        x, ss = x.contiguous(), ss.contiguous()
        out = torch.empty_like(x)
        with torch.cuda.device(x.device):
            _hip_call("ixtts_ln_modulate_f32", x.data_ptr(), ss.data_ptr(), out.data_ptr(), B, T, H, C.c_float(eps))
        return out
    return F.layer_norm(x, (H,), None, None, eps) * (1 + ss[:, None, H:]) + ss[:, None, :H]


def swiglu(u):
    Fd = u.shape[-1] // 2
    if u.is_cuda:
        u = u.contiguous()
        out = torch.empty(*u.shape[:-1], Fd, device=u.device, dtype=u.dtype)
        with torch.cuda.device(u.device):
            _hip_call("ixtts_swiglu_f32", u.data_ptr(), out.data_ptr(), u.numel() // (2 * Fd), Fd)
        return out
    return F.silu(u[..., :Fd]) * u[..., Fd:]


def wn_gate(a, g, off, C_):
    B, _, T = a.shape
    if a.is_cuda:
        a, g = a.contiguous(), g.contiguous()
        out = torch.empty(B, C_, T, device=a.device, dtype=a.dtype)
        with torch.cuda.device(a.device):
            _hip_call("ixtts_wn_gate_f32", a.data_ptr(), g.data_ptr(), out.data_ptr(), B, C_, T, g.shape[1], off)
        return out
    x = a + g[:, off:off + 2 * C_, None]
    return torch.tanh(x[:, :C_]) * torch.sigmoid(x[:, C_:])


def wn_gate_rows(a, g, off, C_, rows_per_batch):
    rows, B = a.shape[0], g.shape[0]
    if a.is_cuda:
        a, g = a.contiguous(), g.contiguous()
        out = torch.empty(rows, C_, device=a.device, dtype=a.dtype)
        with torch.cuda.device(a.device):
            _hip_call("ixtts_wn_gate_rows_f32", a.data_ptr(), g.data_ptr(), out.data_ptr(), rows, C_, rows_per_batch, B, g.shape[1], off)
        return out
    b = (torch.arange(rows, device=a.device) // rows_per_batch).clamp(max=B - 1)
    x = a + g[b, off:off + 2 * C_]
    return torch.tanh(x[:, :C_]) * torch.sigmoid(x[:, C_:])


def reflect_halo_rows(p, T, left, right):
    B, _, C_ = p.shape
    if p.is_cuda:
        assert p.is_contiguous()
        with torch.cuda.device(p.device):
            _hip_call("ixtts_reflect_halo_rows_f32", p.data_ptr(), B, T, C_, left, right)
        return p
    if left:
        p[:, :left] = p[:, left + 1:2 * left + 1].flip(1)
    if right:
        p[:, left + T:] = p[:, left + T - 1 - right:left + T - 1].flip(1)
    return p


class RowPack:

    def __init__(self, lens, device):
        self.lens = [int(t) for t in lens]
        assert self.lens and min(self.lens) >= 1, self.lens
        self.n = len(self.lens)
        self.off = [0]
        for t in self.lens:
            self.off.append(self.off[-1] + t)
        self.rows = self.off[-1]
        self.device = torch.device(device)
        tiles = [0]
        for t in self.lens:
            tiles.append(tiles[-1] + (t + 63) // 64)
        self.tiles = tiles[-1]
        work = [(s, q) for s, t in enumerate(self.lens) for q in range((t + 127) // 128)]
        self.n_work = len(work)
        host = torch.tensor(self.off + tiles + [v for w in work for v in w], dtype=torch.int32)
        self.tab = host.to(self.device)
        if self.device.type != "cuda":
            self.seq = torch.repeat_interleave(torch.arange(self.n), torch.tensor(self.lens))
            self.pos = torch.arange(self.rows) - torch.tensor(self.off[:-1])[self.seq]

    def span(self, s):
        return self.off[s], self.off[s + 1]


def adaln_rmsnorm_packed(x, wb, g, pk, eps=1e-5):
    rows, H = x.shape
    if x.is_cuda:
        import ctypes as C

        x, wb = x.contiguous(), wb.contiguous()
        out = torch.empty_like(x)
        with torch.cuda.device(x.device):
            _hip_call("ixtts_adaln_rmsnorm_varlen_f32", x.data_ptr(), wb.data_ptr(), g.data_ptr(), out.data_ptr(), pk.tab.data_ptr(), pk.n, rows, H, C.c_float(eps))
        return out
    wbr = wb[pk.seq]
    return torch.addcmul(wbr[:, H:], wbr[:, :H], F.rms_norm(x, (H,), g, eps))


def ln_modulate_packed(x, ss, pk, eps=1e-6):
    rows, H = x.shape
    if x.is_cuda:
        import ctypes as C

        x, ss = x.contiguous(), ss.contiguous()
        out = torch.empty_like(x)
        with torch.cuda.device(x.device):
            _hip_call("ixtts_ln_modulate_varlen_f32", x.data_ptr(), ss.data_ptr(), out.data_ptr(), pk.tab.data_ptr(), pk.n, rows, H, C.c_float(eps))
        return out
    ssr = ss[pk.seq]
    return F.layer_norm(x, (H,), None, None, eps) * (1 + ssr[:, H:]) + ssr[:, :H]


def rope_qk_packed(qkv, fc, pk, head_dim):
    rows, H3 = qkv.shape
    H = H3 // 3
    if qkv.is_cuda:
        assert qkv.is_contiguous() and fc.shape[0] >= max(pk.lens)
        with torch.cuda.device(qkv.device):
            _hip_call("ixtts_rope_qk_varlen_f32", qkv.data_ptr(), torch.view_as_real(fc).data_ptr(), pk.tab.data_ptr(), pk.n, rows, H, head_dim)
        return qkv
    f = fc[pk.pos][:, None, :]
    out = qkv.clone()
    for j in range(2):
        xc = torch.view_as_complex(qkv[:, j * H:(j + 1) * H].reshape(rows, H // head_dim, head_dim // 2, 2).contiguous())
        out[:, j * H:(j + 1) * H] = torch.view_as_real(xc * f).reshape(rows, H)
    return out


def attn_full_packed(q, k, v, pk, scale=None):
    import ctypes as C

    from . import _lib

    rows, Hh, d = q.shape
    assert d == 64 and q.is_cuda and q.dtype == torch.float32 and k.shape == q.shape and v.shape == q.shape and rows == pk.rows
    for t in (q, k, v):
        assert t.stride(2) == 1 and t.stride() == q.stride() and t.stride(0) % 4 == 0 and t.data_ptr() % 16 == 0
    out = torch.empty(rows, Hh, d, device=q.device, dtype=torch.float32)
    sc = float(scale if scale is not None else 1.0 / math.sqrt(d))
    L = _lib.lib()
    nws = L.ixtts_attn_full_varlen_workspace_bytes(pk.n, Hh, pk.tiles)
    ws = torch.empty(nws, device=q.device, dtype=torch.uint8)
    with torch.cuda.device(q.device):
        rc = L.ixtts_attn_full_varlen_f32(q.data_ptr(), k.data_ptr(), v.data_ptr(), out.data_ptr(), pk.tab.data_ptr(), pk.n, pk.tiles, pk.n_work, Hh, d,
                                          q.stride(0), q.stride(1), out.stride(0), out.stride(1), C.c_float(sc), ws.data_ptr(), nws, _lib.current_stream_ptr())
    _lib.check(rc, "ixtts_attn_full_varlen_f32")
    return out


def wn_gate_rows_packed(a, g, off, C_, poff):
    rows = a.shape[0]
    if a.is_cuda:
        a, g = a.contiguous(), g.contiguous()
        out = torch.empty(rows, C_, device=a.device, dtype=a.dtype)
        with torch.cuda.device(a.device):
            _hip_call("ixtts_wn_gate_rows_varlen_f32", a.data_ptr(), g.data_ptr(), out.data_ptr(), rows, C_, poff.tab.data_ptr(), poff.n, g.shape[1], off)
        return out
    b = torch.cat([poff.seq, poff.seq.new_full((max(0, rows - poff.rows),), poff.n - 1)])[:rows]
    x = a + g[b, off:off + 2 * C_]
    return torch.tanh(x[:, :C_]) * torch.sigmoid(x[:, C_:])


def _reflect_src(T, left, right):
    idx = _pad_reflect(torch.arange(1, T + 1, dtype=torch.float64)[None, None], left, right)[0, 0].long() - 1
    dst = list(range(left)) + list(range(left + T, left + T + right))
    return dst, [int(idx[i]) + left if int(idx[i]) >= 0 else -1 for i in dst]


def reflect_halo_rows_packed(p, poff, left, right):
    if p.is_cuda:
        assert p.is_contiguous() and min(poff.lens) - left - right > max(left, right)
        with torch.cuda.device(p.device):
            _hip_call("ixtts_reflect_halo_rows_varlen_f32", p.data_ptr(), poff.tab.data_ptr(), poff.n, p.shape[1], left, right)
        return p
    if not hasattr(poff, "halo"):
        dst, src, zero = [], [], []
        for s, L in enumerate(poff.lens):
            o = poff.off[s]
            for d_, s_ in zip(*_reflect_src(L - left - right, left, right)):
                (dst.append(o + d_), src.append(o + s_)) if s_ >= 0 else zero.append(o + d_)
        poff.halo = (torch.tensor(dst, dtype=torch.long), torch.tensor(src, dtype=torch.long), torch.tensor(zero, dtype=torch.long))
    dst, src, zero = poff.halo
    p[dst] = p[src]
    if zero.numel():
        p[zero] = 0
    return p


S2MEL_BATCH_FRAMES = 16384

TUNED_GEMMS = os.path.join(os.path.dirname(os.path.abspath(__file__)), "tunable", "gfx950_s2mel.csv")


def use_tuned_gemms(path=TUNED_GEMMS):
    if not torch.cuda.is_available():
        return False
    import torch.cuda.tunable as tn

    tn.enable(True)
    tn.tuning_enable(os.environ.get("IXTTS_TUNE") == "1")
    try:
        import tempfile

        tn.set_filename(os.path.join(tempfile.gettempdir(), "ixtts_tunableop_online.csv"))
    except Exception:
        pass
    try:
        return bool(os.path.isfile(path) and tn.read_file(path))
    except Exception:
        return False


_TUNED_T0, _TUNED_TH0 = 2322, 1909
_tuned_lengths = set()


def extend_tuned_gemms(T, Th, path=TUNED_GEMMS):
    if (T, Th) in _tuned_lengths or (T, Th) == (_TUNED_T0, _TUNED_TH0):
        return False
    _tuned_lengths.add((T, Th))
    import tempfile

    import torch.cuda.tunable as tn

    sub = {str(2 * _TUNED_T0): str(2 * T), str(_TUNED_T0): str(T), str(_TUNED_TH0): str(Th), str(2 * _TUNED_TH0): str(2 * Th),
           str(2 * _TUNED_TH0 + 4): str(2 * Th + 4)}
    head, rows = [], []
    for line in open(path).read().splitlines():
        f = line.split(",")
        if f[0] == "Validator":
            head.append(line)
        elif len(f) >= 4 and f[2] != "Default" and f[0].endswith("_TN"):
            toks = f[1].split("_")
            if any(t in sub for t in toks):
                rows.append(",".join([f[0], "_".join(sub.get(t, t) for t in toks)] + f[2:]))
    if not rows:
        return False
    with tempfile.NamedTemporaryFile("w", suffix=".csv", delete=False) as fh:
        fh.write("\n".join(head + rows) + "\n")
    try:
        return bool(tn.read_file(fh.name))
    except Exception:
        return False
    finally:
        os.unlink(fh.name)


class S2Mel:
    def __init__(self, W, cfg=S2MEL_CFG, device="cpu"):
        self.cfg = dict(cfg)
        self.device = torch.device(device)
        self.tuned_gemms = False
        if self.device.type == "cuda" and os.environ.get("IXTTS_NO_TUNED_GEMMS") != "1":
            self.tuned_gemms = use_tuned_gemms()
        W = fold_weight_norm(dict(W))
        self.W = {k: v.to(self.device, torch.float32) for k, v in W.items()}
        H = cfg["hidden_dim"]
        self.head_dim = H // cfg["num_heads"]
        half = 128
        self.t_freqs = torch.exp(-math.log(10000.0) * torch.arange(half, dtype=torch.float32) / half).to(self.device)
        self._rope = None
        W, C_, L = self.W, cfg["in_channels"], cfg["depth"]
        t = "cfm.estimator.transformer."
        self.w13 = [torch.cat([W[t + f"layers.{i}.feed_forward.w1.weight"], W[t + f"layers.{i}.feed_forward.w3.weight"]], 0).contiguous() for i in range(L)]
        self.skip_w = {i: (W[t + f"layers.{i}.skip_in_linear.weight"][:, :H].contiguous(), W[t + f"layers.{i}.skip_in_linear.weight"][:, H:].contiguous())
                       for i in range(L // 2 + 1, L)}
        names = [t + f"layers.{i}.{n}" for i in range(L) for n in ("attention_norm", "ffn_norm")] + [t + "norm"]
        self.proj_w = torch.cat([W[n + ".project_layer.weight"] for n in names], 0).contiguous()
        self.proj_b = torch.cat([W[n + ".project_layer.bias"] for n in names], 0).contiguous()
        mw = W["cfm.estimator.cond_x_merge_linear.weight"]
        self.merge_x, self.merge_rest = mw[:, :C_].contiguous(), mw[:, C_:].contiguous()
        wn = "cfm.estimator.wavenet."
        self.wn_taps = [[W[wn + f"in_layers.{i}.conv.conv.weight"][:, :, j].contiguous() for j in range(cfg["wavenet_kernel"])]
                        for i in range(cfg["wavenet_layers"])]
        nl, Hw = cfg["wavenet_layers"], cfg["wavenet_hidden"]
        self.wn_r1, self.wn_r2, self.wn_bin = [], [], []
        carry = torch.zeros(Hw, device=self.device)
        self.wn_out_bias = torch.zeros(Hw, device=self.device)
        for i in range(nl):
            rw, rb = W[wn + f"res_skip_layers.{i}.conv.conv.weight"][:, :, 0], W[wn + f"res_skip_layers.{i}.conv.conv.bias"]
            self.wn_bin.append(W[wn + f"in_layers.{i}.conv.conv.bias"] + sum(self.wn_taps[i]) @ carry)
            if i < nl - 1:
                self.wn_r1.append(rw[:Hw].contiguous())
                self.wn_r2.append(rw[Hw:].contiguous())
                carry = carry + rb[:Hw]
                self.wn_out_bias = self.wn_out_bias + rb[Hw:]
            else:
                self.wn_r1.append(None)
                self.wn_r2.append(rw.contiguous())
                self.wn_out_bias = self.wn_out_bias + rb
        sw = W["cfm.estimator.skip_linear.weight"]
        self.skipl_res, self.skipl_x = sw[:, :H].contiguous(), sw[:, H:].contiguous()
        self.x6_w13, self.x6_wn = None, None
        if self.device.type == "cuda" and H % 64 == 0:
            inter = self.w13[0].shape[0] // 2
            self.x6_w13 = [G.PackedLinear(G.interleave_halves(w[:inter], w[inter:])) for w in self.w13]
            self.x6_wn = [G.PackedLinear(G.interleave_halves(torch.cat(tp, 1)[:Hw], torch.cat(tp, 1)[Hw:]), G.interleave_halves(b[:Hw], b[Hw:]))
                          for tp, b in zip(self.wn_taps, self.wn_bin)]

    def _x6(self, packs):
        return packs is not None and os.environ.get("IXTTS_S2MEL_GEMM", "x6") != "library"

    def gpt_layer(self, latent):
        x = _lin(latent, self.W, "gpt_layer.0")
        x = _lin(x, self.W, "gpt_layer.1")
        return _lin(x, self.W, "gpt_layer.2")

    def vq2emb(self, codes):
        emb = self.W["quantizer.codebook.weight"][codes.long()]
        out = conv1d(emb.transpose(1, 2), self.W["quantizer.out_project.weight"], self.W["quantizer.out_project.bias"])
        return out.transpose(1, 2)

    def length_regulator(self, x, ylens):
        W = self.W
        x = _lin(x, W, "length_regulator.content_in_proj")
        T = int(ylens.max())
        x = F.interpolate(x.transpose(1, 2).contiguous(), size=T, mode="nearest")
        for i in range(self.cfg["lr_n_blocks"]):
            x = conv1d(x, W[f"length_regulator.model.{3 * i}.weight"], W[f"length_regulator.model.{3 * i}.bias"], padding=1)
            x = F.group_norm(x, 1, W[f"length_regulator.model.{3 * i + 1}.weight"], W[f"length_regulator.model.{3 * i + 1}.bias"], 1e-5)
            x = F.mish(x)
        n = 3 * self.cfg["lr_n_blocks"]
        x = conv1d(x, W[f"length_regulator.model.{n}.weight"], W[f"length_regulator.model.{n}.bias"])
        mask = (torch.arange(T, device=x.device).unsqueeze(0) < ylens.unsqueeze(1)).unsqueeze(-1)
        return x.transpose(1, 2) * mask

    def _t_embed(self, t, prefix):
        args = 1000.0 * t[:, None].float() * self.t_freqs[None]
        emb = torch.cat([torch.cos(args), torch.sin(args)], dim=-1)
        h = F.silu(_lin(emb, self.W, prefix + ".mlp.0"))
        return _lin(h, self.W, prefix + ".mlp.2")

    def _rope_cache(self, T):
        if self._rope is None or self._rope.shape[0] < T:
            n = self.head_dim
            freqs = 1.0 / (10000.0 ** (torch.arange(0, n, 2)[: n // 2].float() / n))
            ang = torch.outer(torch.arange(max(T, 64)).float(), freqs)
            self._rope = torch.polar(torch.ones_like(ang), ang).to(self.device)
        return self._rope[:T]

    @staticmethod
    def _rotary(x, fc):
        xc = torch.view_as_complex(x.reshape(*x.shape[:-1], -1, 2))
        return torch.view_as_real(xc * fc.view(1, fc.shape[0], 1, fc.shape[1])).flatten(3)

    def _attention(self, qkv, B, T, mask):
        H, nh, hd = self.cfg["hidden_dim"], self.cfg["num_heads"], self.head_dim
        fc = self._rope_cache(T)
        if mask is None and hd == 64 and qkv.is_cuda:
            with torch.cuda.device(qkv.device):
                _hip_call("ixtts_rope_qk_f32", qkv.data_ptr(), torch.view_as_real(fc).data_ptr(), B, T, H, hd)
            v4 = qkv.view(B, T, 3, nh, hd)
            return attn_full(v4[:, :, 0], v4[:, :, 1], v4[:, :, 2]).reshape(B * T, H)
        q, k, v = qkv.view(B, T, 3 * H).split([H, H, H], dim=-1)
        q = self._rotary(q.reshape(B, T, nh, hd), fc)
        k = self._rotary(k.reshape(B, T, nh, hd), fc)
        v = v.reshape(B, T, nh, hd)
        y = F.scaled_dot_product_attention(q.transpose(1, 2), k.transpose(1, 2), v.transpose(1, 2), attn_mask=mask, dropout_p=0.0)
        return y.transpose(1, 2).reshape(B * T, H)

    def _transformer(self, x, c, mask):
        W, cfg = self.W, self.cfg
        B, T, H = x.shape
        L = cfg["depth"]
        wb_all = F.linear(c, self.proj_w, self.proj_b).view(B, 2 * L + 1, 2 * H).transpose(0, 1).contiguous()
        x = x.reshape(B * T, H)
        x6 = x.is_cuda and self._x6(self.x6_w13)
        skips = []
        for i in range(L):
            p = f"cfm.estimator.transformer.layers.{i}."
            if i > L // 2:
                wa, wb_ = self.skip_w[i]
                x = F.linear(skips.pop(), wb_, W[p + "skip_in_linear.bias"]).addmm_(x, wa.t())
            a = adaln_rmsnorm(x.view(B, T, H), wb_all[2 * i], W[p + "attention_norm.norm.weight"])
            y = self._attention(F.linear(a.view(B * T, H), W[p + "attention.wqkv.weight"]), B, T, mask)
            h = torch.addmm(x, y, W[p + "attention.wo.weight"].t()) if 0 < i <= L // 2 else x.addmm_(y, W[p + "attention.wo.weight"].t())
            f = adaln_rmsnorm(h.view(B, T, H), wb_all[2 * i + 1], W[p + "ffn_norm.norm.weight"]).view(B * T, H)
            u = G.pair_linear(f, self.x6_w13[i], G.SWIGLU) if x6 else swiglu(F.linear(f, self.w13[i]))
            x = h.addmm_(u, W[p + "feed_forward.w2.weight"].t())
            if i < L // 2:
                skips.append(x)
        return adaln_rmsnorm(x.view(B, T, H), wb_all[2 * L], W["cfm.estimator.transformer.norm.norm.weight"])

    def _wavenet(self, x, x_mask, g, full):
        W, cfg = self.W, self.cfg
        Hw, nl, k = cfg["wavenet_hidden"], cfg["wavenet_layers"], cfg["wavenet_kernel"]
        p = "cfm.estimator.wavenet."
        g = F.linear(g, W[p + "cond_layer.conv.conv.weight"][:, :, 0], W[p + "cond_layer.conv.conv.bias"])
        out = None
        for i in range(nl):
            d = cfg["wavenet_dilation_rate"] ** i
            tot = (k - 1) * d
            right = tot // 2
            xin = _pad_reflect(x, tot - right, right)
            if x.is_cuda:
                wk, T_ = self.wn_taps[i], x.shape[-1]
                acc = W[p + f"in_layers.{i}.conv.conv.bias"][None, :, None].expand(x.shape[0], -1, T_)
                for j in range(k):
                    wj, xj = wk[j].expand(x.shape[0], -1, -1), xin[:, :, j * d:j * d + T_]
                    acc = torch.baddbmm(acc, wj, xj) if j == 0 else acc.baddbmm_(wj, xj)
                xin = acc
            else:
                xin = conv1d(xin, W[p + f"in_layers.{i}.conv.conv.weight"], W[p + f"in_layers.{i}.conv.conv.bias"], dilation=d)
            acts = wn_gate(xin, g, i * 2 * Hw, Hw)
            rs = conv1d(acts, W[p + f"res_skip_layers.{i}.conv.conv.weight"], W[p + f"res_skip_layers.{i}.conv.conv.bias"])
            if i < nl - 1:
                x = x + rs[:, :Hw]
                if not full:
                    x = x * x_mask
                out = rs[:, Hw:] if out is None else out + rs[:, Hw:]
            else:
                out = rs if out is None else out + rs
        return out if full else out * x_mask

    def _wavenet_gemm(self, x, g):
        W, cfg = self.W, self.cfg
        Hw, nl, k = cfg["wavenet_hidden"], cfg["wavenet_layers"], cfg["wavenet_kernel"]
        B, _, T_ = x.shape
        p = "cfm.estimator.wavenet."
        g = F.linear(g, W[p + "cond_layer.conv.conv.weight"][:, :, 0], W[p + "cond_layer.conv.conv.bias"])
        x = x.contiguous()
        out = None
        for i in range(nl):
            d = cfg["wavenet_dilation_rate"] ** i
            tot = (k - 1) * d
            right = tot // 2
            xin = _pad_reflect(x, tot - right, right)
            acc = self.wn_bin[i][None, :, None].expand(B, -1, T_)
            for j in range(k):
                wj, xj = self.wn_taps[i][j].expand(B, -1, -1), xin[:, :, j * d:j * d + T_]
                acc = torch.baddbmm(acc, wj, xj) if j == 0 else acc.baddbmm_(wj, xj)
            acts = wn_gate(acc, g, i * 2 * Hw, Hw)
            if i < nl - 1:
                x = x.baddbmm_(self.wn_r1[i].expand(B, -1, -1), acts)
            r2 = self.wn_r2[i].expand(B, -1, -1)
            out = torch.bmm(r2, acts) if out is None else out.baddbmm_(r2, acts)
        return out

    def _wavenet_rows(self, h, g):
        W, cfg = self.W, self.cfg
        Hw, nl, k = cfg["wavenet_hidden"], cfg["wavenet_layers"], cfg["wavenet_kernel"]
        assert cfg["wavenet_dilation_rate"] == 1
        B, T_, _ = h.shape
        p = "cfm.estimator.wavenet."
        g = F.linear(g, W[p + "cond_layer.conv.conv.weight"][:, :, 0], W[p + "cond_layer.conv.conv.bias"])
        tot = k - 1
        right = tot // 2
        left = tot - right
        Tp = T_ + tot
        P = torch.empty(B, Tp, Hw, device=h.device, dtype=h.dtype)
        P[:, left:left + T_] = h
        P2 = P.view(B * Tp, Hw)
        M = B * Tp - tot
        centre = P2[left:left + M]
        out = torch.empty(B * Tp, Hw, device=h.device, dtype=h.dtype)
        x6 = self._x6(self.x6_wn)
        for i in range(nl):
            reflect_halo_rows(P, T_, left, right)
            if x6:
                acts = G.pair_linear(G.split(P2), self.x6_wn[i], G.GATE, taps=k, gate=g, gate_off=i * 2 * Hw, rows_per_batch=Tp)
            else:
                acc = torch.addmm(self.wn_bin[i], P2[:M], self.wn_taps[i][0].t())
                for j in range(1, k):
                    acc.addmm_(P2[j:j + M], self.wn_taps[i][j].t())
                acts = wn_gate_rows(acc, g, i * 2 * Hw, Hw, Tp)
            if i < nl - 1:
                centre.addmm_(acts, self.wn_r1[i].t())
            if i == 0:
                torch.mm(acts, self.wn_r2[i].t(), out=out[:M])
            else:
                out[:M].addmm_(acts, self.wn_r2[i].t())
        return out.view(B, Tp, Hw)[:, :T_]

    def dit_prepare(self, prompt_x, x_lens, style, cond):
        W = self.W
        e = "cfm.estimator."
        B, _, T = prompt_x.shape
        cond = _lin(cond, W, e + "cond_projection")
        rest = torch.cat([prompt_x.transpose(1, 2), cond, style[:, None, :].expand(B, T, style.shape[-1])], dim=-1)
        base = F.linear(rest, self.merge_rest, W[e + "cond_x_merge_linear.bias"])
        x_mask = (torch.arange(T, device=prompt_x.device).unsqueeze(0) < x_lens.unsqueeze(1)).unsqueeze(1)
        full = int(x_lens.min()) >= T
        if full:
            attn_mask = None
        else:
            attn_mask = x_mask[:, None, :].expand(x_mask.shape[0], 1, T, T)
            if attn_mask.shape[0] != B:
                attn_mask = attn_mask.expand(B, 1, T, T)
        return dict(B=B, T=T, base=base, x_mask=x_mask.to(base.dtype), attn_mask=attn_mask, full=full)

    def dit_step(self, ctx, x, t, out_from=0):
        W, cfg = self.W, self.cfg
        e = "cfm.estimator."
        B, T, base = ctx["B"], ctx["T"], ctx["base"]
        xt = x.transpose(1, 2)
        t1 = self._t_embed(t, e + "t_embedder")
        x_in = base + F.linear(xt, self.merge_x)
        x_res = self._transformer(x_in, t1, ctx["attn_mask"])
        halo = sum((cfg["wavenet_kernel"] - 1) * cfg["wavenet_dilation_rate"] ** i for i in range(cfg["wavenet_layers"])) // 2 + 1
        lo = max(0, out_from - halo) if (ctx["full"] and out_from > 0) else 0
        if lo > 0:
            x_res, xt = x_res[:, lo:], xt[:, lo:]
        Th = T - lo
        if self.tuned_gemms and os.environ.get("IXTTS_TUNED_ANY_LENGTH", "1") == "1":
            extend_tuned_gemms(T, Th)
        x_res = F.linear(x_res, self.skipl_res, W[e + "skip_linear.bias"]) + F.linear(xt, self.skipl_x)
        h = _lin(x_res, W, e + "conv1")
        t2 = self._t_embed(t, e + "t_embedder2")
        gemm_form = h.is_cuda and ctx["full"] and Th > 2 * cfg["wavenet_kernel"] * cfg["wavenet_dilation_rate"] ** (cfg["wavenet_layers"] - 1)
        if gemm_form and cfg["wavenet_dilation_rate"] == 1:
            h = self._wavenet_rows(h, t2) + F.linear(x_res, W[e + "res_projection.weight"], W[e + "res_projection.bias"] + self.wn_out_bias)
        elif gemm_form:
            h = self._wavenet_gemm(h.transpose(1, 2), t2).transpose(1, 2) + F.linear(x_res, W[e + "res_projection.weight"],
                                                                                     W[e + "res_projection.bias"] + self.wn_out_bias)
        else:
            mask = ctx["x_mask"][:, :, lo:] if lo > 0 else ctx["x_mask"]
            h = self._wavenet(h.transpose(1, 2), mask, t2, ctx["full"]).transpose(1, 2) + _lin(x_res, W, e + "res_projection")
        ss = _lin(F.silu(t1), W, e + "final_layer.adaLN_modulation.1")
        h = ln_modulate(h, ss)
        h = _lin(h, W, e + "final_layer.linear").transpose(1, 2)
        out = conv1d(h, W[e + "conv2.weight"], W[e + "conv2.bias"])
        return out[:, :, out_from - lo:] if out_from > 0 else out

    def dit(self, x, prompt_x, x_lens, t, style, cond):
        return self.dit_step(self.dit_prepare(prompt_x, x_lens, style, cond), x, t)

    @torch.no_grad()
    def cfm_inference(self, mu, x_lens, prompt, style, n_timesteps=25, inference_cfg_rate=0.7, noise=None, temperature=1.0):
        B, T = mu.shape[0], mu.shape[1]
        assert B == 1, "CFM inference is batch-1 (as the reference)"
        z = (torch.randn(B, self.cfg["in_channels"], T, device=mu.device) if noise is None else noise.to(mu.device, torch.float32)) * temperature
        t_span = torch.linspace(0, 1, n_timesteps + 1, device=mu.device)
        x = z.clone()
        Tp = prompt.shape[-1]
        prompt_x = torch.zeros_like(x)
        prompt_x[..., :Tp] = prompt[..., :Tp]
        x[..., :Tp] = 0
        if inference_cfg_rate > 0:
            ctx = self.dit_prepare(torch.cat([prompt_x, torch.zeros_like(prompt_x)], 0), x_lens, torch.cat([style, torch.zeros_like(style)], 0),
                                   torch.cat([mu, torch.zeros_like(mu)], 0))
        else:
            ctx = self.dit_prepare(prompt_x, x_lens, style, mu)
        t = t_span[0]
        skip = Tp if ctx["full"] else 0
        for step in range(1, len(t_span)):
            dt = t_span[step] - t_span[step - 1]
            if inference_cfg_rate > 0:
                d = self.dit_step(ctx, x, torch.stack([t, t]), out_from=skip)
                dphi = (1.0 + inference_cfg_rate) * d[0:1] - inference_cfg_rate * d[1:2]
            else:
                dphi = self.dit_step(ctx, x, t.expand(B), out_from=skip)
            if skip > 0:
                x[:, :, skip:] += dt * dphi
            else:
                x = x + dt * dphi
            t = t + dt
            x[:, :, :Tp] = 0
        return x

    @torch.no_grad()
    def __call__(self, latent, codes, code_lens, prompt_condition, ref_mel, style, n_timesteps=25, inference_cfg_rate=0.7, noise=None):
        lat = self.gpt_layer(latent)
        S = self.vq2emb(codes) + lat
        target = (code_lens * 1.72).long()
        cond = self.length_regulator(S, target)
        cat = torch.cat([prompt_condition, cond], dim=1)
        lens = torch.tensor([cat.shape[1]], device=cat.device, dtype=torch.long)
        mel = self.cfm_inference(cat, lens, ref_mel, style, n_timesteps, inference_cfg_rate, noise)
        return mel[:, :, ref_mel.shape[-1]:]

    def _attention_packed(self, qkv, pk):
        H, nh, hd = self.cfg["hidden_dim"], self.cfg["num_heads"], self.head_dim
        if qkv.is_cuda and hd == 64 and os.environ.get("IXTTS_ATTN_FULL", "x3") != "f32":
            rope_qk_packed(qkv, self._rope_cache(max(pk.lens)), pk, hd)
            v4 = qkv.view(pk.rows, 3, nh, hd)
            return attn_full_packed(v4[:, 0], v4[:, 1], v4[:, 2], pk).view(pk.rows, H)
        out = torch.empty(pk.rows, H, device=qkv.device, dtype=qkv.dtype)
        if qkv.is_cuda:
            for s in range(pk.n):
                a, b = pk.span(s)
                out[a:b] = self._attention(qkv[a:b], 1, b - a, None)
            return out
        qk = rope_qk_packed(qkv, self._rope_cache(max(pk.lens)), pk, hd)
        for s in range(pk.n):
            a, b = pk.span(s)
            q, k, v = (qk[a:b, :H], qk[a:b, H:2 * H], qkv[a:b, 2 * H:])
            y = F.scaled_dot_product_attention(*(z.reshape(1, b - a, nh, hd).transpose(1, 2) for z in (q, k, v)), dropout_p=0.0)
            out[a:b] = y.transpose(1, 2).reshape(b - a, H)
        return out

    def _transformer_packed(self, x, c, pk):
        W, cfg = self.W, self.cfg
        H, L = cfg["hidden_dim"], cfg["depth"]
        wb_all = F.linear(c, self.proj_w, self.proj_b).view(pk.n, 2 * L + 1, 2 * H).transpose(0, 1).contiguous()
        x6 = x.is_cuda and self._x6(self.x6_w13)
        skips = []
        for i in range(L):
            p = f"cfm.estimator.transformer.layers.{i}."
            if i > L // 2:
                wa, wb_ = self.skip_w[i]
                x = F.linear(skips.pop(), wb_, W[p + "skip_in_linear.bias"]).addmm_(x, wa.t())
            a = adaln_rmsnorm_packed(x, wb_all[2 * i], W[p + "attention_norm.norm.weight"], pk)
            y = self._attention_packed(F.linear(a, W[p + "attention.wqkv.weight"]), pk)
            h = torch.addmm(x, y, W[p + "attention.wo.weight"].t()) if 0 < i <= L // 2 else x.addmm_(y, W[p + "attention.wo.weight"].t())
            f = adaln_rmsnorm_packed(h, wb_all[2 * i + 1], W[p + "ffn_norm.norm.weight"], pk)
            u = G.pair_linear(f, self.x6_w13[i], G.SWIGLU) if x6 else swiglu(F.linear(f, self.w13[i]))
            x = h.addmm_(u, W[p + "feed_forward.w2.weight"].t())
            if i < L // 2:
                skips.append(x)
        return adaln_rmsnorm_packed(x, wb_all[2 * L], W["cfm.estimator.transformer.norm.norm.weight"], pk)

    def _wavenet_packed(self, h, g, hp):
        W, cfg = self.W, self.cfg
        Hw, nl, k = cfg["wavenet_hidden"], cfg["wavenet_layers"], cfg["wavenet_kernel"]
        assert cfg["wavenet_dilation_rate"] == 1
        p = "cfm.estimator.wavenet."
        g = F.linear(g, W[p + "cond_layer.conv.conv.weight"][:, :, 0], W[p + "cond_layer.conv.conv.bias"])
        tot = k - 1
        right = tot // 2
        left = tot - right
        pp, interior = hp.padded, hp.interior
        P2 = torch.empty(pp.rows, Hw, device=h.device, dtype=h.dtype)
        P2[interior] = h
        M = pp.rows - tot
        centre = P2[left:left + M]
        out = torch.empty(pp.rows, Hw, device=h.device, dtype=h.dtype)
        x6 = h.is_cuda and self._x6(self.x6_wn)
        for i in range(nl):
            reflect_halo_rows_packed(P2, pp, left, right)
            if x6:
                acts = G.pair_linear(G.split(P2), self.x6_wn[i], G.GATE, taps=k, gate=g, gate_off=i * 2 * Hw, seq_off=pp)
            else:
                acc = torch.addmm(self.wn_bin[i], P2[:M], self.wn_taps[i][0].t())
                for j in range(1, k):
                    acc.addmm_(P2[j:j + M], self.wn_taps[i][j].t())
                acts = wn_gate_rows_packed(acc, g, i * 2 * Hw, Hw, pp)
            if i < nl - 1:
                centre.addmm_(acts, self.wn_r1[i].t())
            if i == 0:
                torch.mm(acts, self.wn_r2[i].t(), out=out[:M])
            else:
                out[:M].addmm_(acts, self.wn_r2[i].t())
        return out[interior - left]

    def _halo(self):
        cfg = self.cfg
        return sum((cfg["wavenet_kernel"] - 1) * cfg["wavenet_dilation_rate"] ** i for i in range(cfg["wavenet_layers"])) // 2 + 1

    def packable(self, T, Tp, device=None):
        dev = self.device if device is None else torch.device(device)
        if dev.type != "cuda":
            return True
        cfg = self.cfg
        Th = T - max(0, Tp - self._halo())
        return cfg["wavenet_dilation_rate"] == 1 and Th > 2 * cfg["wavenet_kernel"]

    def _cfm_packed(self, segs, n_timesteps, inference_cfg_rate):
        W, cfg = self.W, self.cfg
        e = "cfm.estimator."
        dev = segs[0]["mu"].device
        C_, H = cfg["in_channels"], cfg["hidden_dim"]
        n = len(segs)
        lens = [s["mu"].shape[1] for s in segs]
        Tps = [min(s["prompt"].shape[-1], T) for s, T in zip(segs, lens)]
        R = sum(lens)
        cfg_on = inference_cfg_rate > 0
        nb = 2 if cfg_on else 1
        pk = RowPack(lens * nb, dev)
        xo = pk.off[:n + 1]
        x = torch.cat([s["z"][0].t() for s in segs], 0).contiguous()
        keep = torch.cat([torch.arange(xo[i] + Tps[i], xo[i + 1]) for i in range(n)]).to(dev)
        pmask = torch.ones(R, 1, device=dev)
        for i in range(n):
            pmask[xo[i]:xo[i] + Tps[i]] = 0
        x.mul_(pmask)
        prompt_rows = torch.zeros(R, C_, device=dev)
        for i, s in enumerate(segs):
            prompt_rows[xo[i]:xo[i] + Tps[i]] = s["prompt"][0, :, :Tps[i]].t()
        mu = torch.cat([s["mu"][0] for s in segs], 0)
        style = torch.cat([s["style"].expand(T, -1) for s, T in zip(segs, lens)], 0)
        rest = torch.cat([prompt_rows, _lin(mu, W, e + "cond_projection"), style], -1)
        if cfg_on:
            rest = torch.cat([rest, torch.cat([torch.zeros_like(prompt_rows), _lin(torch.zeros_like(mu), W, e + "cond_projection"), torch.zeros_like(style)], -1)], 0)
        base = F.linear(rest, self.merge_rest, W[e + "cond_x_merge_linear.bias"])
        halo, k = self._halo(), cfg["wavenet_kernel"]
        los = [max(0, Tp - halo) for Tp in Tps] * nb
        head_lens = [L - lo for L, lo in zip(pk.lens, los)]
        hp = RowPack(head_lens, dev)
        hp.padded = RowPack([t + k - 1 for t in head_lens], dev)
        right = (k - 1) // 2
        left = k - 1 - right
        hidx = torch.cat([torch.arange(pk.off[s] + los[s], pk.off[s + 1]) for s in range(pk.n)])
        hp.interior = torch.cat([torch.arange(hp.padded.off[s] + left, hp.padded.off[s] + left + head_lens[s]) for s in range(pk.n)]).to(dev)
        hrows = hidx.to(dev)
        hx = (hidx - torch.tensor(pk.off[:-1]).repeat_interleave(torch.tensor(head_lens)) +
              torch.tensor(xo[:-1] * nb).repeat_interleave(torch.tensor(head_lens))).to(dev)
        hsel = torch.cat([torch.arange(hp.off[s] + Tps[s % n] - los[s], hp.off[s + 1]) for s in range(pk.n)]).to(dev)
        nkeep = keep.numel()
        t_span = torch.linspace(0, 1, n_timesteps + 1, device=dev)
        t = t_span[0]
        for step in range(1, len(t_span)):
            dt = t_span[step] - t_span[step - 1]
            tt = t.expand(pk.n)
            t1 = self._t_embed(tt, e + "t_embedder")
            x_in = (base.view(nb, R, H) + F.linear(x, self.merge_x)).view(nb * R, H)
            x_res = self._transformer_packed(x_in, t1, pk)
            x_res = x_res.index_select(0, hrows)
            xt = x.index_select(0, hx)
            x_res = F.linear(x_res, self.skipl_res, W[e + "skip_linear.bias"]) + F.linear(xt, self.skipl_x)
            h = _lin(x_res, W, e + "conv1")
            t2 = self._t_embed(tt, e + "t_embedder2")
            h = self._wavenet_packed(h, t2, hp) + F.linear(x_res, W[e + "res_projection.weight"], W[e + "res_projection.bias"] + self.wn_out_bias)
            ss = _lin(F.silu(t1), W, e + "final_layer.adaLN_modulation.1")
            h = ln_modulate_packed(h, ss, hp)
            h = _lin(h, W, e + "final_layer.linear")
            d = F.linear(h.index_select(0, hsel), W[e + "conv2.weight"][:, :, 0], W[e + "conv2.bias"])
            dphi = (1.0 + inference_cfg_rate) * d[:nkeep] - inference_cfg_rate * d[nkeep:] if cfg_on else d
            x.index_add_(0, keep, dt * dphi)
            t = t + dt
            x.mul_(pmask)
        return [x[xo[i]:xo[i + 1]].t()[None] for i in range(n)]

    @torch.no_grad()
    def solve_many(self, items, n_timesteps=25, inference_cfg_rate=0.7, noises=None):
        segs = []
        for i, (latent, codes, prompt_condition, ref_mel, style) in enumerate(items):
            code_lens = torch.tensor([codes.shape[-1]], device=codes.device)
            S = self.vq2emb(codes) + self.gpt_layer(latent)
            cond = self.length_regulator(S, (code_lens * 1.72).long())
            mu = torch.cat([prompt_condition, cond], dim=1)
            T = mu.shape[1]
            z = torch.randn(1, self.cfg["in_channels"], T, device=mu.device) if noises is None or noises[i] is None else \
                noises[i].to(mu.device, torch.float32)
            segs.append(dict(mu=mu, prompt=ref_mel, style=style, z=z, Tp=ref_mel.shape[-1]))
        xs = [None] * len(segs)
        budget = max(1, int(os.environ.get("IXTTS_S2MEL_BATCH_FRAMES", str(S2MEL_BATCH_FRAMES))))
        order = sorted(range(len(segs)), key=lambda i: segs[i]["mu"].shape[1])
        groups, cur, used = [], [], 0
        for i in order:
            T = segs[i]["mu"].shape[1]
            if not self.packable(T, segs[i]["Tp"], segs[i]["mu"].device):
                groups.append([i])
                continue
            if cur and used + T > budget:
                groups.append(cur)
                cur, used = [], 0
            cur.append(i)
            used += T
        if cur:
            groups.append(cur)
        for grp in groups:
            if len(grp) == 1 and not self.packable(segs[grp[0]]["mu"].shape[1], segs[grp[0]]["Tp"], segs[grp[0]]["mu"].device):
                s = segs[grp[0]]
                lens = torch.tensor([s["mu"].shape[1]], device=s["mu"].device, dtype=torch.long)
                xs[grp[0]] = self.cfm_inference(s["mu"], lens, s["prompt"], s["style"], n_timesteps, inference_cfg_rate, s["z"])
                continue
            for i, x in zip(grp, self._cfm_packed([segs[i] for i in grp], n_timesteps, inference_cfg_rate)):
                xs[i] = x
        return [x[:, :, s["Tp"]:] for x, s in zip(xs, segs)]
```

Measured before the change: 40.93.

## Fold RoPE into attention and emit bf16 planes from AdaLN norm for x6 GEMMs

```diff
diff --git a/include/ixtts_hip.h b/include/ixtts_hip.h
--- a/include/ixtts_hip.h
+++ b/include/ixtts_hip.h
@@ -26,13 +26,23 @@
                         int head_dim, long stride_b, long stride_t, long stride_h, long ostride_b, long ostride_t,
                         long ostride_h, float scale, void* workspace_dev, size_t workspace_bytes, void* stream);
 
+int ixtts_attn_full_rope_f32(const float* q_dev, const float* k_dev, const float* v_dev, float* out_dev, const float* cos_sin_dev, int B, int H,
+                             int T, int head_dim, long stride_b, long stride_t, long stride_h, long ostride_b, long ostride_t, long ostride_h,
+                             float scale, void* workspace_dev, size_t workspace_bytes, void* stream);
+
 size_t ixtts_attn_full_varlen_workspace_bytes(int nseq, int H, int total_tiles);
 int ixtts_attn_full_varlen_f32(const float* q_dev, const float* k_dev, const float* v_dev, float* out_dev, const int* table_dev, int nseq,
                                int total_tiles, int n_work, int H, int head_dim, long stride_t, long stride_h, long ostride_t, long ostride_h,
                                float scale, void* workspace_dev, size_t workspace_bytes, void* stream);
 
+int ixtts_attn_full_rope_varlen_f32(const float* q_dev, const float* k_dev, const float* v_dev, float* out_dev, const float* cos_sin_dev,
+                                    const int* table_dev, int nseq, int total_tiles, int n_work, int H, int head_dim, long stride_t, long stride_h,
+                                    long ostride_t, long ostride_h, float scale, void* workspace_dev, size_t workspace_bytes, void* stream);
+
 int ixtts_adaln_rmsnorm_f32(const float* x_dev, const float* wb_dev, const float* g_dev, float* out_dev, int B, int T, int H, float eps,
                             void* stream);
+int ixtts_adaln_rmsnorm_planes_f32(const float* x_dev, const float* wb_dev, const float* g_dev, void* planes_dev, int B, int T, int H, float eps,
+                                   void* stream);
 int ixtts_ln_modulate_f32(const float* x_dev, const float* shift_scale_dev, float* out_dev, int B, int T, int H, float eps, void* stream);
 int ixtts_rope_qk_f32(float* qkv_dev, const float* cos_sin_dev, int B, int T, int H, int head_dim, void* stream);
 int ixtts_swiglu_f32(const float* u_dev, float* out_dev, long rows, int F, void* stream);
@@ -43,6 +53,8 @@
 
 int ixtts_adaln_rmsnorm_varlen_f32(const float* x_dev, const float* wb_dev, const float* g_dev, float* out_dev, const int* seq_off_dev, int nseq,
                                    long rows, int H, float eps, void* stream);
+int ixtts_adaln_rmsnorm_planes_varlen_f32(const float* x_dev, const float* wb_dev, const float* g_dev, void* planes_dev, const int* seq_off_dev,
+                                          int nseq, long rows, int H, float eps, void* stream);
 int ixtts_ln_modulate_varlen_f32(const float* x_dev, const float* shift_scale_dev, float* out_dev, const int* seq_off_dev, int nseq, long rows, int H,
                                  float eps, void* stream);
 int ixtts_rope_qk_varlen_f32(float* qkv_dev, const float* cos_sin_dev, const int* seq_off_dev, int nseq, long rows, int H, int head_dim, void* stream);
diff --git a/voice-tts_amd/_lib.py b/voice-tts_amd/_lib.py
--- a/voice-tts_amd/_lib.py
+++ b/voice-tts_amd/_lib.py
@@ -59,10 +59,15 @@
     "ixtts_attn_full_workspace_bytes": (C.c_size_t, [C.c_int, C.c_int, C.c_int]),
     "ixtts_attn_full_f32": (C.c_int, [_P, _P, _P, _P, C.c_int, C.c_int, C.c_int, C.c_int, C.c_long, C.c_long, C.c_long, C.c_long, C.c_long,
                                       C.c_long, C.c_float, _P, C.c_size_t, _P]),
+    "ixtts_attn_full_rope_f32": (C.c_int, [_P, _P, _P, _P, _P, C.c_int, C.c_int, C.c_int, C.c_int, C.c_long, C.c_long, C.c_long, C.c_long, C.c_long,
+                                           C.c_long, C.c_float, _P, C.c_size_t, _P]),
     "ixtts_attn_full_varlen_workspace_bytes": (C.c_size_t, [C.c_int, C.c_int, C.c_int]),
     "ixtts_attn_full_varlen_f32": (C.c_int, [_P, _P, _P, _P, _P, C.c_int, C.c_int, C.c_int, C.c_int, C.c_int, C.c_long, C.c_long, C.c_long, C.c_long,
                                              C.c_float, _P, C.c_size_t, _P]),
+    "ixtts_attn_full_rope_varlen_f32": (C.c_int, [_P, _P, _P, _P, _P, _P, C.c_int, C.c_int, C.c_int, C.c_int, C.c_int, C.c_long, C.c_long, C.c_long,
+                                                  C.c_long, C.c_float, _P, C.c_size_t, _P]),
     "ixtts_adaln_rmsnorm_f32": (C.c_int, [_P, _P, _P, _P, C.c_int, C.c_int, C.c_int, C.c_float, _P]),
+    "ixtts_adaln_rmsnorm_planes_f32": (C.c_int, [_P, _P, _P, _P, C.c_int, C.c_int, C.c_int, C.c_float, _P]),
     "ixtts_ln_modulate_f32": (C.c_int, [_P, _P, _P, C.c_int, C.c_int, C.c_int, C.c_float, _P]),
     "ixtts_rope_qk_f32": (C.c_int, [_P, _P, C.c_int, C.c_int, C.c_int, C.c_int, _P]),
     "ixtts_swiglu_f32": (C.c_int, [_P, _P, C.c_long, C.c_int, _P]),
@@ -70,6 +75,7 @@
     "ixtts_wn_gate_rows_f32": (C.c_int, [_P, _P, _P, C.c_long, C.c_int, C.c_long, C.c_int, C.c_long, C.c_int, _P]),
     "ixtts_reflect_halo_rows_f32": (C.c_int, [_P, C.c_int, C.c_int, C.c_int, C.c_int, C.c_int, _P]),
     "ixtts_adaln_rmsnorm_varlen_f32": (C.c_int, [_P, _P, _P, _P, _P, C.c_int, C.c_long, C.c_int, C.c_float, _P]),
+    "ixtts_adaln_rmsnorm_planes_varlen_f32": (C.c_int, [_P, _P, _P, _P, _P, C.c_int, C.c_long, C.c_int, C.c_float, _P]),
     "ixtts_ln_modulate_varlen_f32": (C.c_int, [_P, _P, _P, _P, C.c_int, C.c_long, C.c_int, C.c_float, _P]),
     "ixtts_rope_qk_varlen_f32": (C.c_int, [_P, _P, _P, C.c_int, C.c_long, C.c_int, C.c_int, _P]),
     "ixtts_wn_gate_rows_varlen_f32": (C.c_int, [_P, _P, _P, C.c_long, C.c_int, _P, C.c_int, C.c_long, C.c_int, _P]),
diff --git a/voice-tts_amd/csrc/attn_full.h b/voice-tts_amd/csrc/attn_full.h
--- a/voice-tts_amd/csrc/attn_full.h
+++ b/voice-tts_amd/csrc/attn_full.h
@@ -23,6 +23,7 @@
   float* ws_ml;
   const int* vl_tab;
   int vl_n, vl_tiles;
+  const float2* rope;
 };
 
 size_t attn_full_x3_plane_bytes(int B, int H, int T);
diff --git a/voice-tts_amd/csrc/attn_full.hip b/voice-tts_amd/csrc/attn_full.hip
--- a/voice-tts_amd/csrc/attn_full.hip
+++ b/voice-tts_amd/csrc/attn_full.hip
@@ -184,9 +184,9 @@
   return attn_partials_bytes(B, H, T) + ixtts::attn_full_x3_plane_bytes(B, H, T);
 }
 
-extern "C" int ixtts_attn_full_f32(const float* q_dev, const float* k_dev, const float* v_dev, float* out_dev, int B, int H, int T,
-                                   int head_dim, long stride_b, long stride_t, long stride_h, long ostride_b, long ostride_t,
-                                   long ostride_h, float scale, void* workspace_dev, size_t workspace_bytes, void* stream) {
+static int attn_full_run(const float* q_dev, const float* k_dev, const float* v_dev, float* out_dev, const float* cos_sin_dev, int B, int H, int T,
+                         int head_dim, long stride_b, long stride_t, long stride_h, long ostride_b, long ostride_t, long ostride_h, float scale,
+                         void* workspace_dev, size_t workspace_bytes, void* stream) {
   using namespace ixtts;
   IX_ARG(q_dev && k_dev && v_dev && out_dev, "attn_full: null pointer");
   IX_ARG(head_dim == AF_D, "attn_full: head_dim %d (only 64 is built)", head_dim);
@@ -199,6 +199,7 @@
   a.B = B; a.H = H; a.T = T; a.scale = scale;
   a.ws_o = a.ws_ml = nullptr;
   a.vl_tab = nullptr; a.vl_n = a.vl_tiles = 0;
+  a.rope = reinterpret_cast<const float2*>(cos_sin_dev);
   hipStream_t st = (hipStream_t)stream;
   const int qblocks = ceil_div(T, AF_WAVES * AF_QW);
   const bool have_ws = workspace_dev && workspace_bytes >= ixtts_attn_full_workspace_bytes(B, H, T);
@@ -206,6 +207,8 @@
   const char* mode = getenv("IXTTS_ATTN_FULL");
   const bool x3 = !(mode && strcmp(mode, "f32") == 0);
   const bool use_x3 = x3 && have_ws;
+  IX_ARG(!cos_sin_dev || use_x3, "attn_full_rope: the rotation is folded into the bf16-plane kernel only (workspace %s, IXTTS_ATTN_FULL=%s)",
+         have_ws ? "given" : "missing or too small", mode ? mode : "");
   if (split) {
     a.ws_o = reinterpret_cast<float*>(workspace_dev);
     a.ws_ml = a.ws_o + (size_t)(use_x3 ? AX_KSPLIT : AF_KSPLIT) * B * H * T * AF_D;
@@ -230,14 +233,29 @@
   return IXTTS_OK;
 }
 
+extern "C" int ixtts_attn_full_f32(const float* q_dev, const float* k_dev, const float* v_dev, float* out_dev, int B, int H, int T,
+                                   int head_dim, long stride_b, long stride_t, long stride_h, long ostride_b, long ostride_t,
+                                   long ostride_h, float scale, void* workspace_dev, size_t workspace_bytes, void* stream) {
+  return attn_full_run(q_dev, k_dev, v_dev, out_dev, nullptr, B, H, T, head_dim, stride_b, stride_t, stride_h, ostride_b, ostride_t, ostride_h, scale,
+                       workspace_dev, workspace_bytes, stream);
+}
+
+extern "C" int ixtts_attn_full_rope_f32(const float* q_dev, const float* k_dev, const float* v_dev, float* out_dev, const float* cos_sin_dev, int B, int H,
+                                        int T, int head_dim, long stride_b, long stride_t, long stride_h, long ostride_b, long ostride_t,
+                                        long ostride_h, float scale, void* workspace_dev, size_t workspace_bytes, void* stream) {
+  IX_ARG(cos_sin_dev && (reinterpret_cast<uintptr_t>(cos_sin_dev) & 15) == 0, "attn_full_rope: cos/sin table null or not 16-byte aligned");
+  return attn_full_run(q_dev, k_dev, v_dev, out_dev, cos_sin_dev, B, H, T, head_dim, stride_b, stride_t, stride_h, ostride_b, ostride_t, ostride_h, scale,
+                       workspace_dev, workspace_bytes, stream);
+}
+
 extern "C" size_t ixtts_attn_full_varlen_workspace_bytes(int nseq, int H, int total_tiles) {
   if (nseq <= 0 || H <= 0 || total_tiles <= 0) return 0;
   return (size_t)H * total_tiles * 2 * 3 * 8 * 64 * 16;
 }
 
-extern "C" int ixtts_attn_full_varlen_f32(const float* q_dev, const float* k_dev, const float* v_dev, float* out_dev, const int* table_dev, int nseq,
-                                          int total_tiles, int n_work, int H, int head_dim, long stride_t, long stride_h, long ostride_t, long ostride_h,
-                                          float scale, void* workspace_dev, size_t workspace_bytes, void* stream) {
+static int attn_full_varlen_run(const float* q_dev, const float* k_dev, const float* v_dev, float* out_dev, const float* cos_sin_dev, const int* table_dev,
+                                int nseq, int total_tiles, int n_work, int H, int head_dim, long stride_t, long stride_h, long ostride_t, long ostride_h,
+                                float scale, void* workspace_dev, size_t workspace_bytes, void* stream) {
   using namespace ixtts;
   IX_ARG(q_dev && k_dev && v_dev && out_dev && table_dev, "attn_full_varlen: null pointer");
   IX_ARG(head_dim == AF_D, "attn_full_varlen: head_dim %d (only 64 is built)", head_dim);
@@ -253,5 +271,22 @@
   a.B = 1; a.H = H; a.T = 0; a.scale = scale;
   a.ws_o = a.ws_ml = nullptr;
   a.vl_tab = table_dev; a.vl_n = nseq; a.vl_tiles = total_tiles;
+  a.rope = reinterpret_cast<const float2*>(cos_sin_dev);
   return launch_attn_full_x3_varlen(a, workspace_dev, n_work, (hipStream_t)stream);
 }
+
+extern "C" int ixtts_attn_full_varlen_f32(const float* q_dev, const float* k_dev, const float* v_dev, float* out_dev, const int* table_dev, int nseq,
+                                          int total_tiles, int n_work, int H, int head_dim, long stride_t, long stride_h, long ostride_t, long ostride_h,
+                                          float scale, void* workspace_dev, size_t workspace_bytes, void* stream) {
+  return attn_full_varlen_run(q_dev, k_dev, v_dev, out_dev, nullptr, table_dev, nseq, total_tiles, n_work, H, head_dim, stride_t, stride_h, ostride_t,
+                              ostride_h, scale, workspace_dev, workspace_bytes, stream);
+}
+
+extern "C" int ixtts_attn_full_rope_varlen_f32(const float* q_dev, const float* k_dev, const float* v_dev, float* out_dev, const float* cos_sin_dev,
+                                               const int* table_dev, int nseq, int total_tiles, int n_work, int H, int head_dim, long stride_t,
+                                               long stride_h, long ostride_t, long ostride_h, float scale, void* workspace_dev, size_t workspace_bytes,
+                                               void* stream) {
+  IX_ARG(cos_sin_dev && (reinterpret_cast<uintptr_t>(cos_sin_dev) & 15) == 0, "attn_full_rope_varlen: cos/sin table null or not 16-byte aligned");
+  return attn_full_varlen_run(q_dev, k_dev, v_dev, out_dev, cos_sin_dev, table_dev, nseq, total_tiles, n_work, H, head_dim, stride_t, stride_h, ostride_t,
+                              ostride_h, scale, workspace_dev, workspace_bytes, stream);
+}
diff --git a/voice-tts_amd/csrc/attn_full_x3.hip b/voice-tts_amd/csrc/attn_full_x3.hip
--- a/voice-tts_amd/csrc/attn_full_x3.hip
+++ b/voice-tts_amd/csrc/attn_full_x3.hip
@@ -43,7 +43,12 @@
     const int t = t0 + key;
     float v[8];
     const float4* src = reinterpret_cast<const float4*>(kb + (long)min(t, T - 1) * a.st + 8 * oct);
-    const float4 x0 = src[0], x1 = src[1];
+    float4 x0 = src[0], x1 = src[1];
+    if (a.rope) {
+      const float4* f = reinterpret_cast<const float4*>(a.rope + (long)min(t, T - 1) * (AF_D / 2) + 4 * oct);
+      x0 = rope2(x0, f[0]);
+      x1 = rope2(x1, f[1]);
+    }
     const bool live = t < T;
     v[0] = live ? x0.x : 0.f; v[1] = live ? x0.y : 0.f; v[2] = live ? x0.z : 0.f; v[3] = live ? x0.w : 0.f;
     v[4] = live ? x1.x : 0.f; v[5] = live ? x1.y : 0.f; v[6] = live ? x1.z : 0.f; v[7] = live ? x1.w : 0.f;
@@ -106,9 +111,14 @@
     const int qi = min(q0 + l31, T - 1);
     const float* qrow = qb + (long)qi * a.st + 8 * lh;
     const float qs = a.scale * 1.4426950408889634f;
+    const float4* frow = reinterpret_cast<const float4*>(a.rope + (long)qi * (AF_D / 2) + 4 * lh);
 #pragma unroll
     for (int s = 0; s < 4; ++s) {
-      const float4 x0 = *reinterpret_cast<const float4*>(qrow + 16 * s), x1 = *reinterpret_cast<const float4*>(qrow + 16 * s + 4);
+      float4 x0 = *reinterpret_cast<const float4*>(qrow + 16 * s), x1 = *reinterpret_cast<const float4*>(qrow + 16 * s + 4);
+      if (a.rope) {
+        x0 = rope2(x0, frow[4 * s]);
+        x1 = rope2(x1, frow[4 * s + 1]);
+      }
       const float v[8] = {x0.x * qs, x0.y * qs, x0.z * qs, x0.w * qs, x1.x * qs, x1.y * qs, x1.z * qs, x1.w * qs};
       split8_bf16x3(v, qp[s][0], qp[s][1], qp[s][2]);
     }
diff --git a/voice-tts_amd/csrc/common.h b/voice-tts_amd/csrc/common.h
--- a/voice-tts_amd/csrc/common.h
+++ b/voice-tts_amd/csrc/common.h
@@ -138,4 +138,9 @@
   pl = make_uint4(pk(l[1], l[0]), pk(l[3], l[2]), pk(l[5], l[4]), pk(l[7], l[6]));
 }
 
+__device__ __forceinline__ float4 rope2(float4 v, float4 f) {
+  return make_float4(__builtin_fmaf(v.x, f.x, -(v.y * f.y)), __builtin_fmaf(v.y, f.x, v.x * f.y), __builtin_fmaf(v.z, f.z, -(v.w * f.w)),
+                     __builtin_fmaf(v.w, f.z, v.z * f.w));
 }
+
+}
diff --git a/voice-tts_amd/csrc/dit_ops.hip b/voice-tts_amd/csrc/dit_ops.hip
--- a/voice-tts_amd/csrc/dit_ops.hip
+++ b/voice-tts_amd/csrc/dit_ops.hip
@@ -5,11 +5,9 @@
 constexpr int ROW_NV = 8;
 
 template <bool CENTER>
-__global__ __launch_bounds__(256) void row_norm_mod_kernel(const float* __restrict__ x, const float* __restrict__ mw, const float* __restrict__ mb,
-                                                           const float* __restrict__ g, float* __restrict__ out, long rows, int T, int H, long mstride,
-                                                           float eps, float wadd, const int* __restrict__ seq_off = nullptr, int nseq = 0) {
-  const long row = (long)blockIdx.x * 4 + (threadIdx.x >> 6);
-  if (row >= rows) return;
+__device__ __forceinline__ void row_norm_mod_row(const float* __restrict__ x, const float* __restrict__ mw, const float* __restrict__ mb,
+                                                 const float* __restrict__ g, float* __restrict__ dst, long row, int T, int H, long mstride, float eps,
+                                                 float wadd, const int* __restrict__ seq_off, int nseq) {
   const int lane = threadIdx.x & 63;
   const int H4 = H >> 2;
   const float4* xr = reinterpret_cast<const float4*>(x + row * H);
@@ -40,7 +38,7 @@
   const float4* w4 = reinterpret_cast<const float4*>(mw + bidx * mstride);
   const float4* b4 = reinterpret_cast<const float4*>(mb + bidx * mstride);
   const float4* g4 = reinterpret_cast<const float4*>(g);
-  float4* o4 = reinterpret_cast<float4*>(out + row * H);
+  float4* o4 = reinterpret_cast<float4*>(dst);
 #pragma unroll
   for (int i = 0; i < ROW_NV; ++i) {
     const int c = lane + 64 * i;
@@ -56,6 +54,45 @@
   }
 }
 
+constexpr int RNP_ROWS = 8;
+
+template <bool CENTER, bool PLANES = false>
+__global__ __launch_bounds__(256) void row_norm_mod_kernel(const float* __restrict__ x, const float* __restrict__ mw, const float* __restrict__ mb,
+                                                           const float* __restrict__ g, float* __restrict__ out, long rows, int T, int H, long mstride,
+                                                           float eps, float wadd, const int* __restrict__ seq_off = nullptr, int nseq = 0, long Mpad = 0) {
+  if constexpr (!PLANES) {
+    const long row = (long)blockIdx.x * 4 + (threadIdx.x >> 6);
+    if (row >= rows) return;
+    row_norm_mod_row<CENTER>(x, mw, mb, g, out + row * H, row, T, H, mstride, eps, wadd, seq_off, nseq);
+  } else {
+    extern __shared__ float rnp_tile[];
+    const int ld = H + 4;
+    const long r0 = (long)blockIdx.x * RNP_ROWS;
+#pragma unroll
+    for (int j = 0; j < RNP_ROWS / 4; ++j) {
+      const int r = (threadIdx.x >> 6) * (RNP_ROWS / 4) + j;
+      if (r0 + r < rows) row_norm_mod_row<CENTER>(x, mw, mb, g, rnp_tile + r * ld, r0 + r, T, H, mstride, eps, wadd, seq_off, nseq);
+    }
+    __syncthreads();
+    uint4* planes = reinterpret_cast<uint4*>(out);
+    const int r = threadIdx.x & (RNP_ROWS - 1);
+    const bool live = r0 + r < rows;
+    for (int ko = threadIdx.x / RNP_ROWS; ko < (H >> 3); ko += 256 / RNP_ROWS) {
+      uint4 ph = make_uint4(0u, 0u, 0u, 0u), pm = ph, pl = ph;
+      if (live) {
+        const float4 a = *reinterpret_cast<const float4*>(rnp_tile + r * ld + 8 * ko), b = *reinterpret_cast<const float4*>(rnp_tile + r * ld + 8 * ko + 4);
+        const float v[8] = {a.x, a.y, a.z, a.w, b.x, b.y, b.z, b.w};
+        split8_bf16x3(v, ph, pm, pl);
+      }
+      const int gk = ko >> 1, kh = ko & 1;
+      uint4* base = planes + ((long)gk * 6) * Mpad + r0 + r;
+      base[(long)(0 * 2 + kh) * Mpad] = ph;
+      base[(long)(1 * 2 + kh) * Mpad] = pm;
+      base[(long)(2 * 2 + kh) * Mpad] = pl;
+    }
+  }
+}
+
 __global__ __launch_bounds__(256) void rope_qk_kernel(float* __restrict__ qkv, const float2* __restrict__ tab, long rows, int T, int H, int hd,
                                                       const int* __restrict__ seq_off = nullptr, int nseq = 0) {
   const int per_row = (2 * H) >> 2;
@@ -69,7 +106,7 @@
   float4* ptr = reinterpret_cast<float4*>(qkv + row * 3 * H + col);
   const float4 v = *ptr;
   const float2 f0 = tab[(long)t * (hd >> 1) + p], f1 = tab[(long)t * (hd >> 1) + p + 1];
-  *ptr = make_float4(v.x * f0.x - v.y * f0.y, v.y * f0.x + v.x * f0.y, v.z * f1.x - v.w * f1.y, v.w * f1.x + v.z * f1.y);
+  *ptr = rope2(v, make_float4(f0.x, f0.y, f1.x, f1.y));
 }
 
 __global__ __launch_bounds__(256) void swiglu_kernel(const float* __restrict__ u, float* __restrict__ out, long rows, int Fd) {
@@ -163,6 +200,25 @@
   return IXTTS_OK;
 }
 
+static int launch_adaln_planes(const float* x, const float* wb, const float* g, void* planes, long rows, int T, int H, float eps, const int* seq_off, int nseq,
+                               hipStream_t st) {
+  IX_ARG(H % 64 == 0 && (reinterpret_cast<uintptr_t>(planes) & 15) == 0, "adaln_rmsnorm_planes: H %d must be a multiple of 64 and the planes 16-byte aligned", H);
+  const long Mpad = ixtts_gemm_x6_rows_padded(rows);
+  const size_t smem = (size_t)RNP_ROWS * (H + 4) * sizeof(float);
+  IX_ARG(smem <= 64 * 1024, "adaln_rmsnorm_planes: H %d needs %zu bytes of LDS", H, smem);
+  hipLaunchKernelGGL((row_norm_mod_kernel<false, true>), dim3((unsigned)(Mpad / RNP_ROWS)), dim3(256), smem, st, x, wb, wb + H, g, reinterpret_cast<float*>(planes),
+                     rows, T, H, (long)2 * H, eps, 0.0f, seq_off, nseq, Mpad);
+  IX_HIP(hipGetLastError());
+  return IXTTS_OK;
+}
+
+extern "C" int ixtts_adaln_rmsnorm_planes_f32(const float* x_dev, const float* wb_dev, const float* g_dev, void* planes_dev, int B, int T, int H, float eps,
+                                              void* stream) {
+  IX_ARG(x_dev && wb_dev && g_dev && planes_dev, "adaln_rmsnorm_planes: null pointer");
+  IX_ARG(B > 0 && T > 0 && H > 0 && H <= 64 * ROW_NV * 4, "adaln_rmsnorm_planes: bad shape B=%d T=%d H=%d", B, T, H);
+  return launch_adaln_planes(x_dev, wb_dev, g_dev, planes_dev, (long)B * T, T, H, eps, nullptr, 0, (hipStream_t)stream);
+}
+
 extern "C" int ixtts_ln_modulate_f32(const float* x_dev, const float* shift_scale_dev, float* out_dev, int B, int T, int H, float eps, void* stream) {
   IX_ARG(x_dev && shift_scale_dev && out_dev, "ln_modulate: null pointer");
   IX_ARG(B > 0 && T > 0 && H > 0 && H % 4 == 0 && H <= 64 * ROW_NV * 4, "ln_modulate: bad shape B=%d T=%d H=%d", B, T, H);
@@ -235,6 +291,13 @@
   return IXTTS_OK;
 }
 
+extern "C" int ixtts_adaln_rmsnorm_planes_varlen_f32(const float* x_dev, const float* wb_dev, const float* g_dev, void* planes_dev, const int* seq_off_dev,
+                                                     int nseq, long rows, int H, float eps, void* stream) {
+  IX_ARG(x_dev && wb_dev && g_dev && planes_dev && seq_off_dev, "adaln_rmsnorm_planes_varlen: null pointer");
+  IX_ARG(nseq > 0 && rows > 0 && H > 0 && H <= 64 * ROW_NV * 4, "adaln_rmsnorm_planes_varlen: bad shape nseq=%d rows=%ld H=%d", nseq, rows, H);
+  return launch_adaln_planes(x_dev, wb_dev, g_dev, planes_dev, rows, 1, H, eps, seq_off_dev, nseq, (hipStream_t)stream);
+}
+
 extern "C" int ixtts_ln_modulate_varlen_f32(const float* x_dev, const float* shift_scale_dev, float* out_dev, const int* seq_off_dev, int nseq, long rows, int H,
                                             float eps, void* stream) {
   IX_ARG(x_dev && shift_scale_dev && out_dev && seq_off_dev, "ln_modulate_varlen: null pointer");
diff --git a/voice-tts_amd/gemm.py b/voice-tts_amd/gemm.py
--- a/voice-tts_amd/gemm.py
+++ b/voice-tts_amd/gemm.py
@@ -37,20 +37,25 @@
         (x.dim() == 1 or (x.stride(-2) % 4 == 0 and x.stride(-2) >= K))
 
 
+def empty_planes(device, rows, K, slot=0):
+    assert K % 64 == 0, K
+    nbytes = (K // 16) * 6 * int(_lib.lib().ixtts_gemm_x6_rows_padded(rows)) * 16
+    key = (device, nbytes, slot)
+    buf = _POOL.get(key)
+    if buf is None:
+        buf = _POOL[key] = torch.empty(nbytes, dtype=torch.uint8, device=device)
+    return Planes(buf, rows, K)
+
+
 def split(x, slot=0):
     K = int(x.shape[-1])
     if x.dim() != 2:
         x = x.reshape(-1, K) if x.is_contiguous() else x.contiguous().reshape(-1, K)
     rows, lda = int(x.shape[0]), int(x.stride(0))
-    L = _lib.lib()
-    nbytes = (K // 16) * 6 * int(L.ixtts_gemm_x6_rows_padded(rows)) * 16
-    key = (x.device, nbytes, slot)
-    buf = _POOL.get(key)
-    if buf is None:
-        buf = _POOL[key] = torch.empty(nbytes, dtype=torch.uint8, device=x.device)
+    pl = empty_planes(x.device, rows, K, slot)
     with torch.cuda.device(x.device):
-        _lib.check(L.ixtts_gemm_x6_split(x.data_ptr(), lda, buf.data_ptr(), rows, K, _lib.current_stream_ptr()), "ixtts_gemm_x6_split")
-    return Planes(buf, rows, K)
+        _lib.check(_lib.lib().ixtts_gemm_x6_split(x.data_ptr(), lda, pl.buf.data_ptr(), rows, K, _lib.current_stream_ptr()), "ixtts_gemm_x6_split")
+    return pl
 
 
 def linear(x, pl, out=None, accumulate=False, bias=True, tile=0, row0=0, rows=None, lead=None):
diff --git a/voice-tts_amd/s2mel.py b/voice-tts_amd/s2mel.py
--- a/voice-tts_amd/s2mel.py
+++ b/voice-tts_amd/s2mel.py
@@ -101,7 +101,10 @@
     return y[..., : y.shape[-1] - extra]
 
 
-def attn_full(q, k, v, scale=None):
+WQKV_X6_MIN_ROWS = 2689
+
+
+def attn_full(q, k, v, scale=None, rope=None):
     import ctypes as C
 
     from . import _lib
@@ -115,11 +118,15 @@
     L = _lib.lib()
     nws = L.ixtts_attn_full_workspace_bytes(B, Hh, T)
     ws = torch.empty(nws, device=q.device, dtype=torch.uint8)
+    tail = (B, Hh, T, d, q.stride(0), q.stride(1), q.stride(2), out.stride(0), out.stride(1), out.stride(2), C.c_float(sc), ws.data_ptr(), nws,
+            _lib.current_stream_ptr())
     with torch.cuda.device(q.device):
-        rc = L.ixtts_attn_full_f32(q.data_ptr(), k.data_ptr(), v.data_ptr(), out.data_ptr(), B, Hh, T, d, q.stride(0), q.stride(1),
-                                   q.stride(2), out.stride(0), out.stride(1), out.stride(2), C.c_float(sc), ws.data_ptr(), nws,
-                                   _lib.current_stream_ptr())
-    _lib.check(rc, "ixtts_attn_full_f32")
+        if rope is None:
+            _lib.check(L.ixtts_attn_full_f32(q.data_ptr(), k.data_ptr(), v.data_ptr(), out.data_ptr(), *tail), "ixtts_attn_full_f32")
+        else:
+            assert rope.is_cuda and rope.dtype == torch.complex64 and rope.is_contiguous() and rope.shape[0] >= T and rope.shape[1] == d // 2
+            _lib.check(L.ixtts_attn_full_rope_f32(q.data_ptr(), k.data_ptr(), v.data_ptr(), out.data_ptr(), torch.view_as_real(rope).data_ptr(), *tail),
+                       "ixtts_attn_full_rope_f32")
     return out
 
 
@@ -133,12 +140,17 @@
     _lib.check(getattr(_lib.lib(), name)(*args, _lib.current_stream_ptr()), name)
 
 
-def adaln_rmsnorm(x, wb, g, eps=1e-5):
+def adaln_rmsnorm(x, wb, g, eps=1e-5, planes=False):
     B, T, H = x.shape
     if x.is_cuda:
         import ctypes as C
 
         x, wb = x.contiguous(), wb.contiguous()
+        if planes:
+            pl = G.empty_planes(x.device, B * T, H)
+            with torch.cuda.device(x.device):
+                _hip_call("ixtts_adaln_rmsnorm_planes_f32", x.data_ptr(), wb.data_ptr(), g.data_ptr(), pl.buf.data_ptr(), B, T, H, C.c_float(eps))
+            return pl
         out = torch.empty_like(x)
         with torch.cuda.device(x.device):
             _hip_call("ixtts_adaln_rmsnorm_f32", x.data_ptr(), wb.data_ptr(), g.data_ptr(), out.data_ptr(), B, T, H, C.c_float(eps))
@@ -237,12 +249,18 @@
         return self.off[s], self.off[s + 1]
 
 
-def adaln_rmsnorm_packed(x, wb, g, pk, eps=1e-5):
+def adaln_rmsnorm_packed(x, wb, g, pk, eps=1e-5, planes=False):
     rows, H = x.shape
     if x.is_cuda:
         import ctypes as C
 
         x, wb = x.contiguous(), wb.contiguous()
+        if planes:
+            pl = G.empty_planes(x.device, rows, H)
+            with torch.cuda.device(x.device):
+                _hip_call("ixtts_adaln_rmsnorm_planes_varlen_f32", x.data_ptr(), wb.data_ptr(), g.data_ptr(), pl.buf.data_ptr(), pk.tab.data_ptr(), pk.n, rows, H,
+                          C.c_float(eps))
+            return pl
         out = torch.empty_like(x)
         with torch.cuda.device(x.device):
             _hip_call("ixtts_adaln_rmsnorm_varlen_f32", x.data_ptr(), wb.data_ptr(), g.data_ptr(), out.data_ptr(), pk.tab.data_ptr(), pk.n, rows, H, C.c_float(eps))
@@ -281,7 +299,7 @@
     return out
 
 
-def attn_full_packed(q, k, v, pk, scale=None):
+def attn_full_packed(q, k, v, pk, scale=None, rope=None):
     import ctypes as C
 
     from . import _lib
@@ -295,10 +313,15 @@
     L = _lib.lib()
     nws = L.ixtts_attn_full_varlen_workspace_bytes(pk.n, Hh, pk.tiles)
     ws = torch.empty(nws, device=q.device, dtype=torch.uint8)
+    tail = (pk.tab.data_ptr(), pk.n, pk.tiles, pk.n_work, Hh, d, q.stride(0), q.stride(1), out.stride(0), out.stride(1), C.c_float(sc), ws.data_ptr(), nws,
+            _lib.current_stream_ptr())
     with torch.cuda.device(q.device):
-        rc = L.ixtts_attn_full_varlen_f32(q.data_ptr(), k.data_ptr(), v.data_ptr(), out.data_ptr(), pk.tab.data_ptr(), pk.n, pk.tiles, pk.n_work, Hh, d,
-                                          q.stride(0), q.stride(1), out.stride(0), out.stride(1), C.c_float(sc), ws.data_ptr(), nws, _lib.current_stream_ptr())
-    _lib.check(rc, "ixtts_attn_full_varlen_f32")
+        if rope is None:
+            _lib.check(L.ixtts_attn_full_varlen_f32(q.data_ptr(), k.data_ptr(), v.data_ptr(), out.data_ptr(), *tail), "ixtts_attn_full_varlen_f32")
+        else:
+            assert rope.is_cuda and rope.dtype == torch.complex64 and rope.is_contiguous() and rope.shape[0] >= max(pk.lens) and rope.shape[1] == d // 2
+            _lib.check(L.ixtts_attn_full_rope_varlen_f32(q.data_ptr(), k.data_ptr(), v.data_ptr(), out.data_ptr(), torch.view_as_real(rope).data_ptr(), *tail),
+                       "ixtts_attn_full_rope_varlen_f32")
     return out
 
 
@@ -445,15 +468,20 @@
                 self.wn_out_bias = self.wn_out_bias + rb
         sw = W["cfm.estimator.skip_linear.weight"]
         self.skipl_res, self.skipl_x = sw[:, :H].contiguous(), sw[:, H:].contiguous()
-        self.x6_w13, self.x6_wn = None, None
+        self.x6_w13, self.x6_wn, self.x6_wqkv = None, None, None
         if self.device.type == "cuda" and H % 64 == 0:
             inter = self.w13[0].shape[0] // 2
+            self.x6_wqkv = [G.PackedLinear(W[f"cfm.estimator.transformer.layers.{i}.attention.wqkv.weight"]) for i in range(len(self.w13))]
             self.x6_w13 = [G.PackedLinear(G.interleave_halves(w[:inter], w[inter:])) for w in self.w13]
             self.x6_wn = [G.PackedLinear(G.interleave_halves(torch.cat(tp, 1)[:Hw], torch.cat(tp, 1)[Hw:]), G.interleave_halves(b[:Hw], b[Hw:]))
                           for tp, b in zip(self.wn_taps, self.wn_bin)]
 
     def _x6(self, packs):
         return packs is not None and os.environ.get("IXTTS_S2MEL_GEMM", "x6") != "library"
+
+    @staticmethod
+    def _fold_rope():
+        return os.environ.get("IXTTS_S2MEL_GEMM", "x6") != "library" and os.environ.get("IXTTS_ATTN_FULL", "x3") != "f32"
 
     def gpt_layer(self, latent):
         x = _lin(latent, self.W, "gpt_layer.0")
@@ -502,9 +530,11 @@
         H, nh, hd = self.cfg["hidden_dim"], self.cfg["num_heads"], self.head_dim
         fc = self._rope_cache(T)
         if mask is None and hd == 64 and qkv.is_cuda:
+            v4 = qkv.view(B, T, 3, nh, hd)
+            if self._fold_rope():
+                return attn_full(v4[:, :, 0], v4[:, :, 1], v4[:, :, 2], rope=fc).reshape(B * T, H)
             with torch.cuda.device(qkv.device):
                 _hip_call("ixtts_rope_qk_f32", qkv.data_ptr(), torch.view_as_real(fc).data_ptr(), B, T, H, hd)
-            v4 = qkv.view(B, T, 3, nh, hd)
             return attn_full(v4[:, :, 0], v4[:, :, 1], v4[:, :, 2]).reshape(B * T, H)
         q, k, v = qkv.view(B, T, 3 * H).split([H, H, H], dim=-1)
         q = self._rotary(q.reshape(B, T, nh, hd), fc)
@@ -520,17 +550,19 @@
         wb_all = F.linear(c, self.proj_w, self.proj_b).view(B, 2 * L + 1, 2 * H).transpose(0, 1).contiguous()
         x = x.reshape(B * T, H)
         x6 = x.is_cuda and self._x6(self.x6_w13)
+        x6_qkv = x6 and B * T >= WQKV_X6_MIN_ROWS
         skips = []
         for i in range(L):
             p = f"cfm.estimator.transformer.layers.{i}."
             if i > L // 2:
                 wa, wb_ = self.skip_w[i]
                 x = F.linear(skips.pop(), wb_, W[p + "skip_in_linear.bias"]).addmm_(x, wa.t())
-            a = adaln_rmsnorm(x.view(B, T, H), wb_all[2 * i], W[p + "attention_norm.norm.weight"])
-            y = self._attention(F.linear(a.view(B * T, H), W[p + "attention.wqkv.weight"]), B, T, mask)
+            a = adaln_rmsnorm(x.view(B, T, H), wb_all[2 * i], W[p + "attention_norm.norm.weight"], planes=x6_qkv)
+            qkv = G.linear(a, self.x6_wqkv[i], tile=3) if x6_qkv else F.linear(a.view(B * T, H), W[p + "attention.wqkv.weight"])
+            y = self._attention(qkv, B, T, mask)
             h = torch.addmm(x, y, W[p + "attention.wo.weight"].t()) if 0 < i <= L // 2 else x.addmm_(y, W[p + "attention.wo.weight"].t())
-            f = adaln_rmsnorm(h.view(B, T, H), wb_all[2 * i + 1], W[p + "ffn_norm.norm.weight"]).view(B * T, H)
-            u = G.pair_linear(f, self.x6_w13[i], G.SWIGLU) if x6 else swiglu(F.linear(f, self.w13[i]))
+            f = adaln_rmsnorm(h.view(B, T, H), wb_all[2 * i + 1], W[p + "ffn_norm.norm.weight"], planes=x6)
+            u = G.pair_linear(f, self.x6_w13[i], G.SWIGLU) if x6 else swiglu(F.linear(f.view(B * T, H), self.w13[i]))
             x = h.addmm_(u, W[p + "feed_forward.w2.weight"].t())
             if i < L // 2:
                 skips.append(x)
@@ -726,8 +758,11 @@
     def _attention_packed(self, qkv, pk):
         H, nh, hd = self.cfg["hidden_dim"], self.cfg["num_heads"], self.head_dim
         if qkv.is_cuda and hd == 64 and os.environ.get("IXTTS_ATTN_FULL", "x3") != "f32":
-            rope_qk_packed(qkv, self._rope_cache(max(pk.lens)), pk, hd)
+            fc = self._rope_cache(max(pk.lens))
             v4 = qkv.view(pk.rows, 3, nh, hd)
+            if self._fold_rope():
+                return attn_full_packed(v4[:, 0], v4[:, 1], v4[:, 2], pk, rope=fc).view(pk.rows, H)
+            rope_qk_packed(qkv, fc, pk, hd)
             return attn_full_packed(v4[:, 0], v4[:, 1], v4[:, 2], pk).view(pk.rows, H)
         out = torch.empty(pk.rows, H, device=qkv.device, dtype=qkv.dtype)
         if qkv.is_cuda:
@@ -748,16 +783,17 @@
         H, L = cfg["hidden_dim"], cfg["depth"]
         wb_all = F.linear(c, self.proj_w, self.proj_b).view(pk.n, 2 * L + 1, 2 * H).transpose(0, 1).contiguous()
         x6 = x.is_cuda and self._x6(self.x6_w13)
+        x6_qkv = x6 and pk.rows >= WQKV_X6_MIN_ROWS
         skips = []
         for i in range(L):
             p = f"cfm.estimator.transformer.layers.{i}."
             if i > L // 2:
                 wa, wb_ = self.skip_w[i]
                 x = F.linear(skips.pop(), wb_, W[p + "skip_in_linear.bias"]).addmm_(x, wa.t())
-            a = adaln_rmsnorm_packed(x, wb_all[2 * i], W[p + "attention_norm.norm.weight"], pk)
-            y = self._attention_packed(F.linear(a, W[p + "attention.wqkv.weight"]), pk)
+            a = adaln_rmsnorm_packed(x, wb_all[2 * i], W[p + "attention_norm.norm.weight"], pk, planes=x6_qkv)
+            y = self._attention_packed(G.linear(a, self.x6_wqkv[i], tile=3) if x6_qkv else F.linear(a, W[p + "attention.wqkv.weight"]), pk)
             h = torch.addmm(x, y, W[p + "attention.wo.weight"].t()) if 0 < i <= L // 2 else x.addmm_(y, W[p + "attention.wo.weight"].t())
-            f = adaln_rmsnorm_packed(h, wb_all[2 * i + 1], W[p + "ffn_norm.norm.weight"], pk)
+            f = adaln_rmsnorm_packed(h, wb_all[2 * i + 1], W[p + "ffn_norm.norm.weight"], pk, planes=x6)
             u = G.pair_linear(f, self.x6_w13[i], G.SWIGLU) if x6 else swiglu(F.linear(f, self.w13[i]))
             x = h.addmm_(u, W[p + "feed_forward.w2.weight"].t())
             if i < L // 2:
```

Measured after the change: 40.99 (median of 2 runs). Within noise of the previous version (+0.1%).
